# hagabbar/GenNet

Hardware: AMD Instinct MI355X
Metric: waveforms/sec (CNN+GAN step, 2048-sample BBH) (higher is better)
Workload: dtype f32

## Files before the change

### gennet_amd/csrc/capi.hip

```cpp
#include <stdarg.h>
#include <algorithm>
#include <mutex>
#include <vector>
#include <stdlib.h>
#include "common.h"

namespace gn {

static thread_local char g_err[512] = "";

void set_error(const char* fmt, ...) {
  va_list ap;
  va_start(ap, fmt);
  vsnprintf(g_err, sizeof(g_err), fmt, ap);
  va_end(ap);
}

int check_launch(const char* what) {
  hipError_t e = hipGetLastError();
  if (e != hipSuccess) {
    set_error("%s: %s", what, hipGetErrorString(e));
    return GN_ELAUNCH;
  }
  return GN_OK;
}

struct ProfRec {
  hipEvent_t a, b;
  double flop;
  int kind;
  double bytes;
};
static bool g_prof_on = false;
static std::vector<ProfRec> g_prof;
static std::vector<hipEvent_t> g_pool;
static hipEvent_t g_cur;
static std::mutex g_prof_mu;

static hipEvent_t get_event() {
  if (!g_pool.empty()) {
    hipEvent_t e = g_pool.back();
    g_pool.pop_back();
    return e;
  }
  hipEvent_t e;
  (void)hipEventCreate(&e);
  return e;
}

static thread_local const uint64_t* g_rng_base = nullptr;
const uint64_t* rng_base() { return g_rng_base; }

void prof_begin(hipStream_t s) {
  if (!g_prof_on) return;
  g_cur = get_event();
  (void)hipEventRecord(g_cur, s);
}

void prof_end(hipStream_t s, double flop, int kind, double bytes) {
  if (!g_prof_on) return;
  hipEvent_t b = get_event();
  (void)hipEventRecord(b, s);
  std::lock_guard<std::mutex> lk(g_prof_mu);
  g_prof.push_back({g_cur, b, flop, kind, bytes});
}

const Switches& switches() {
  static const Switches sw = [] {
    auto on = [](const char* name) { return getenv(name) != nullptr; };
    const char* gflop = getenv("GN_BF16X3_MIN_GFLOP");
    return Switches{on("GN_CONV_NOPIPE"),  on("GN_CONV_NODMA"),   on("GN_CONV_NOMERGE"),    on("GN_CONV_NONARROW"), on("GN_CONV_NOPATCH"),
                    on("GN_WGRAD_NOPIPE"), on("GN_BF16X3_NO_MERGE"), gflop ? atof(gflop) : 50.0};
  }();
  return sw;
}

static int g_conv_math = 0;
static void* g_conv_ws = nullptr;
static size_t g_conv_ws_bytes = 0;
constexpr size_t kWinoKernelBytes = 64ull << 20;

static bool split_worth_it(int B, int M, int ntaps, int Cin, int Cout) {
  constexpr int min_cin = 256, min_cout = 256;
  return Cin >= min_cin && Cout >= min_cout && 2.0 * B * (double)M * ntaps * Cin * Cout >= switches().bf16x3_min_gflop * 1e9;
}
static bool split_worth_it(const ConvArgs& a, int w_taps) {
  return w_taps > 0 ? split_worth_it(a.B, (a.Ly + 1) / 2, w_taps, a.Cin, a.Cout) : split_worth_it(a.B, a.M, a.t.ntaps, a.Cin, a.Cout);
}

static bool needs_any(int Cin, int Cout) {
  const bool strict = Cin <= 4 ? Cout % 4 == 0 : Cout <= 4 ? Cin % 4 == 0 : (Cin % 4 == 0 && Cout % 4 == 0);
  return !strict;
}

enum ConvFamily { CONV_SMALL, CONV_WINO, CONV_WINO_S2, CONV_BF16X3, CONV_DIRECT, CONV_ANYC };

static ConvFamily select_conv(const ConvArgs& a, int w_taps) {
  if (a.any_channels && needs_any(a.Cin, a.Cout)) return CONV_ANYC;
  if (a.Cin <= 4 || a.Cout <= 4) return CONV_SMALL;
  if (g_conv_math == 2 && a.Cin >= 32 && conv_wino_supported(a) && conv_wino_workspace_bytes(a.Cin, a.Cout) <= kWinoKernelBytes) return CONV_WINO;
  if (g_conv_math == 2 && conv_wino_s2_kind(a) == 1 && conv_wino_s2_workspace_bytes(a.Cin, a.Cout) <= kWinoKernelBytes) return CONV_WINO_S2;
  if (g_conv_math == 1 && split_worth_it(a, w_taps) && conv_bf16x3_supported(a)) return CONV_BF16X3;
  return CONV_DIRECT;
}

enum DgradFamily { DGRAD_WINO_S2, DGRAD_BF16X3_MERGED, DGRAD_MERGED, DGRAD_PHASES };

static DgradFamily select_dgrad(const ConvArgs& a) {
  if (a.any_channels && needs_any(a.Cin, a.Cout)) return DGRAD_PHASES;
  if (a.Ly < 2 || a.Cin <= 4 || a.Cout <= 4) return DGRAD_PHASES;
  if (g_conv_math == 2 && conv_wino_s2_kind(a) == 2 && conv_wino_s2_workspace_bytes(a.Cin, a.Cout) <= kWinoKernelBytes) return DGRAD_WINO_S2;
  const Switches& sw = switches();
  const bool split = g_conv_math == 1 && split_worth_it(a, 5);
  if (split) return !sw.bf16x3_no_merge && conv_bf16x3_merged_kind(a) ? DGRAD_BF16X3_MERGED : DGRAD_PHASES;
  if (!sw.conv_nomerge && !sw.conv_nopipe && !sw.conv_nodma && conv_pipe_merged_supported(a)) return DGRAD_MERGED;
  return DGRAD_PHASES;
}

enum WgradFamily { WGRAD_SMALL, WGRAD_WINO, WGRAD_WINO_S2, WGRAD_BF16X3, WGRAD_DIRECT, WGRAD_ANYC };

static WgradFamily select_wgrad(const WgradArgs& a) {
  if (a.any_channels && needs_any(a.Cin, a.Cout)) return WGRAD_ANYC;
  if (a.Cin <= 4 || a.Cout <= 4) return WGRAD_SMALL;
  if (g_conv_math == 2 && wgrad_wino_supported(a) && conv_wino_workspace_bytes(a.Cin, a.Cout) <= kWinoKernelBytes) return WGRAD_WINO;
  if (g_conv_math == 2 && wgrad_wino_s2_supported(a) && conv_wino_s2_workspace_bytes(a.Cin, a.Cout) <= kWinoKernelBytes) return WGRAD_WINO_S2;
  if (g_conv_math == 1 && split_worth_it(a.B, a.M, a.ntaps, a.Cin, a.Cout) && wgrad_bf16x3_supported(a)) return WGRAD_BF16X3;
  return WGRAD_DIRECT;
}

static size_t wgrad_ws_need(WgradFamily f, const WgradArgs& a) {
  switch (f) {
    case WGRAD_SMALL: return needs_any(a.Cin, a.Cout) ? 0 : wgrad_small_workspace_bytes(a.B, a.M, a.Cin, a.Cout, a.ntaps);
    case WGRAD_WINO: return wgrad_wino_workspace_bytes(a.B, a.M, a.Cin, a.Cout);
    case WGRAD_WINO_S2: return wgrad_wino_s2_workspace_bytes(a.B, a.M, a.Cin, a.Cout);
    case WGRAD_ANYC: return wgrad_anyc_workspace_bytes(a.B, a.M, a.Cin, a.Cout, a.ntaps);
    default: return wgrad_workspace_bytes(a.B, a.M, a.Cin, a.Cout, a.ntaps);
  }
}

static int ws_check(const char* what, size_t need, size_t have) {
  if (need <= have) return GN_OK;
  set_error("%s workspace: the selected kernel needs %zu bytes, the workspace has %zu", what, need, have);
  return GN_EWORKSPACE;
}

struct Phases { int w_taps; bool have_split; };

static int conv_run(const ConvArgs& a, hipStream_t s, Phases* ph = nullptr) {
  const ConvFamily f = select_conv(a, ph ? ph->w_taps : 0);
  int w_taps = ph ? ph->w_taps : 0;
  for (int j = 0; !ph && j < a.t.ntaps; ++j) w_taps = std::max(w_taps, a.t.widx[j] + 1);
  const size_t need = f == CONV_WINO ? conv_wino_workspace_bytes(a.Cin, a.Cout) : f == CONV_WINO_S2 ? conv_wino_s2_workspace_bytes(a.Cin, a.Cout)
                      : f == CONV_BF16X3 ? conv_bf16x3_workspace_bytes(a.B, a.Lin, a.Cin, a.Cout, w_taps) : 0;
  if (int rc = ws_check("conv-math", need, g_conv_ws_bytes)) return rc;
  switch (f) {
    case CONV_SMALL: return a.Cin <= 4 ? conv_smallcin_dispatch(a, s) : conv_smallcout_dispatch(a, s);
    case CONV_WINO: return conv_wino_run(a, g_conv_ws, g_conv_ws_bytes, s);
    case CONV_WINO_S2: return conv_wino_s2_run(a, g_conv_ws, g_conv_ws_bytes, s);
    case CONV_BF16X3:
      if (!(ph && ph->have_split)) {
        int rc = conv_bf16x3_split(a, w_taps, g_conv_ws, g_conv_ws_bytes, true, true, s);
        if (rc) return rc;
        if (ph) ph->have_split = true;
      }
      return conv_bf16x3_run(a, w_taps, g_conv_ws, s);
    case CONV_ANYC: return conv_anyc_dispatch(a, s);
    default: return conv_mfma_dispatch(a, s);
  }
}

static ConvArgs fwd_args(const float* x, const float* w, const float* bias, float* y, int B, int L, int Cin, int Cout, int k, int stride, int pad_left,
                         int Lout, int act, float act_param) {
  ConvArgs a = {};
  a.x = x; a.w = w; a.bias = bias; a.y = y;
  a.B = B; a.Lin = L; a.Cin = Cin; a.Cout = Cout; a.M = Lout; a.Ly = Lout;
  a.t.ntaps = k; a.t.in_stride = stride; a.t.out_stride = 1;
  for (int j = 0; j < k; ++j) { a.t.off[j] = j - pad_left; a.t.widx[j] = j; }
  a.act = act; a.act_param = act_param;
  return a;
}

static int set_conv_math_impl(int mode, void* workspace, size_t workspace_bytes) {
  GN_REQUIRE(mode >= 0 && mode <= 2, "set_conv_math: mode %d (0 = direct fp32, 1 = bf16x3, 2 = transform-domain fp32)", mode);
  GN_REQUIRE(mode == 0 || workspace, "set_conv_math: modes 1 and 2 need a device workspace");
  if (mode == 2 && workspace_bytes < kWinoKernelBytes) {
    set_error("set_conv_math: the transform-domain math needs a workspace of %zu bytes, got %zu", kWinoKernelBytes, workspace_bytes);
    return GN_EWORKSPACE;
  }
  g_conv_math = mode;
  g_conv_ws = mode ? workspace : nullptr;
  g_conv_ws_bytes = mode ? workspace_bytes : 0;
  return GN_OK;
}

__global__ void colsum_anyc_kernel(const float* __restrict__ x, double* __restrict__ acc, size_t n, int C) {
  double s[4] = {0, 0, 0, 0};
  const size_t stride = (size_t)gridDim.x * blockDim.x;
  for (size_t i = (size_t)blockIdx.x * blockDim.x + threadIdx.x; i < n; i += stride) {
    const int c = (int)(i % C);
    const double v = (double)x[i];
    s[0] += c == 0 ? v : 0.0; s[1] += c == 1 ? v : 0.0; s[2] += c == 2 ? v : 0.0; s[3] += c == 3 ? v : 0.0;
  }
  __shared__ double red[4][256];
  for (int c = 0; c < 4; ++c) red[c][threadIdx.x] = s[c];
  __syncthreads();
  for (int sft = 128; sft >= 1; sft >>= 1) {
    if (threadIdx.x < sft)
      for (int c = 0; c < 4; ++c) red[c][threadIdx.x] += red[c][threadIdx.x + sft];
    __syncthreads();
  }
  if (threadIdx.x < C) atomicAdd(&acc[threadIdx.x], red[threadIdx.x][0]);
}
__global__ void f64_to_f32_small_kernel(const double* __restrict__ a, float* __restrict__ o, int n) {
  if ((int)threadIdx.x < n) o[threadIdx.x] = (float)a[threadIdx.x];
}

static int bias_grad(const float* dy, float* db, size_t rows, int C, void* ws, size_t ws_bytes, hipStream_t s) {
  if (C % 4 == 0 || C > 4) {
    ColRedArgs r = {};
    r.a = dy; r.rows = rows; r.C = C;
    return colred_run(0, r, ws, ws_bytes, nullptr, db, s);
  }
  if (ws_bytes < 32) { set_error("bias_grad: workspace too small"); return GN_EWORKSPACE; }
  (void)hipMemsetAsync(ws, 0, 32, s);
  size_t g = (rows * C + 255) / 256;
  if (g > 1024) g = 1024;
  hipLaunchKernelGGL(colsum_anyc_kernel, dim3((unsigned)g), dim3(256), 0, s, dy, (double*)ws, rows * C, C);
  hipLaunchKernelGGL(f64_to_f32_small_kernel, dim3(1), dim3(64), 0, s, (const double*)ws, db, C);
  return check_launch("bias_grad");
}

static size_t bias_grad_ws(size_t rows, int C) { return C % 4 == 0 || C > 4 ? colred_workspace_bytes(rows, C) : 32; }

__global__ __launch_bounds__(256) void dense_any_kernel(const float* __restrict__ A, const float* __restrict__ Bm, const float* __restrict__ bias,
                                                        float* __restrict__ C, int M, int N, int K, size_t sam, size_t sak, size_t sbk, size_t sbn, int act,
                                                        float p) {
  __shared__ float As[16][17], Bs[16][17];
  const int tx = threadIdx.x % 16, ty = threadIdx.x / 16;
  const int m = blockIdx.y * 16 + ty, n = blockIdx.x * 16 + tx;
  float acc = 0.f;
  for (int k0 = 0; k0 < K; k0 += 16) {
    const int ka = k0 + tx, kb = k0 + ty;
    As[ty][tx] = (m < M && ka < K) ? A[(size_t)m * sam + (size_t)ka * sak] : 0.f;
    Bs[ty][tx] = (kb < K && n < N) ? Bm[(size_t)kb * sbk + (size_t)n * sbn] : 0.f;
    __syncthreads();
#pragma unroll
    for (int kk = 0; kk < 16; ++kk) acc = fmaf(As[ty][kk], Bs[kk][tx], acc);
    __syncthreads();
  }
  if (m < M && n < N) C[(size_t)m * N + n] = act_apply(bias ? acc + bias[n] : acc, act, p);
}
static int dense_any_gemm(const float* A, const float* Bm, const float* bias, float* C, int M, int N, int K, size_t sam, size_t sak, size_t sbk, size_t sbn,
                          int act, float p, hipStream_t s) {
  if (M <= 0 || N <= 0) return GN_OK;
  if ((M + 15) / 16 > 65535) { set_error("dense: %d rows exceed the grid", M); return GN_EINVAL; }
  hipLaunchKernelGGL(dense_any_kernel, dim3(cdiv(N, 16), cdiv(M, 16)), dim3(256), 0, s, A, Bm, bias, C, M, N, K, sam, sak, sbk, sbn, act, p);
  return check_launch("dense_any");
}
static bool dense_any_shape(int in, int out) { return (in % 4 || out % 4) && !(out <= 4 && in % 4 == 0); }

}

using namespace gn;

extern "C" {

const char* gn_last_error(void) { return g_err; }
int gn_version(void) { return 100; }

int gn_prof_enable(int on) {
  g_prof_on = on != 0;
  return GN_OK;
}
int gn_prof_reset(void) {
  std::lock_guard<std::mutex> lk(g_prof_mu);
  for (auto& r : g_prof) {
    g_pool.push_back(r.a);
    g_pool.push_back(r.b);
  }
  g_prof.clear();
  return GN_OK;
}
int gn_prof_collect(int kind, double* out) {
  std::lock_guard<std::mutex> lk(g_prof_mu);
  double ms = 0, flop = 0, cnt = 0, bytes = 0;
  for (auto& r : g_prof) {
    if (kind >= 0 && r.kind != kind) continue;
    cnt += 1;
    if (hipEventSynchronize(r.b) != hipSuccess) { set_error("prof: event sync failed"); return GN_ELAUNCH; }
    float t = 0;
    if (hipEventElapsedTime(&t, r.a, r.b) != hipSuccess) { set_error("prof: elapsed failed"); return GN_ELAUNCH; }
    ms += t;
    flop += r.flop;
    bytes += r.bytes;
  }
  out[0] = cnt;
  out[1] = ms;
  out[2] = flop;
  out[3] = bytes;
  return GN_OK;
}

static int fwd_impl(const float* x, const float* w, const float* bias, float* y, int B, int L, int Cin, int Cout, int k, int stride, int pad_left, int Lout,
                    int act, float act_param, bool any_channels, void* stream) {
  GN_REQUIRE(x && w && y, "conv1d_fwd: null pointer");
  GN_REQUIRE(B >= 0 && L > 0 && Cin > 0 && Cout > 0 && k >= 1 && k <= 8 && stride >= 1 && Lout > 0, "conv1d_fwd: bad shape");
  GN_REQUIRE(pad_left >= 0 && stride * (Lout - 1) + k - pad_left <= L + k, "conv1d_fwd: Lout %d inconsistent with L %d k %d stride %d", Lout, L, k, stride);
  if (B == 0) return GN_OK;
  ConvArgs a = fwd_args(x, w, bias, y, B, L, Cin, Cout, k, stride, pad_left, Lout, act, act_param);
  a.any_channels = any_channels;
  return conv_run(a, (hipStream_t)stream);
}

int gn_conv1d_fwd(const float* x, const float* w, const float* bias, float* y, int B, int L, int Cin, int Cout, int k, int stride, int pad_left, int Lout,
                  int act, float act_param, void* stream) {
  return fwd_impl(x, w, bias, y, B, L, Cin, Cout, k, stride, pad_left, Lout, act, act_param, false, stream);
}
int gn_conv1d_fwd_any(const float* x, const float* w, const float* bias, float* y, int B, int L, int Cin, int Cout, int k, int stride, int pad_left, int Lout,
                      int act, float act_param, void* stream) {
  return fwd_impl(x, w, bias, y, B, L, Cin, Cout, k, stride, pad_left, Lout, act, act_param, true, stream);
}
int gn_conv1d_needs_any(int Cin, int Cout) { return needs_any(Cin, Cout) ? 1 : 0; }

int gn_set_conv_math(int mode, void* workspace, size_t workspace_bytes) { return set_conv_math_impl(mode, workspace, workspace_bytes); }

size_t gn_conv1d_bf16x3_workspace(int B, int L, int Cin, int Cout, int k) { return conv_bf16x3_workspace_bytes(B, L, Cin, Cout, k); }

size_t gn_conv1d_fwd_stats_workspace(int B, int Lout, int Cout) {
  const size_t fused = (size_t)B * (size_t)((Lout + 63) / 64) * 2 * (size_t)Cout * sizeof(double);
  const size_t plain = colred_workspace_bytes((size_t)B * Lout, Cout);
  return (fused > plain ? fused : plain) + 256;
}

int gn_conv1d_fwd_stats(const float* x, const float* w, const float* bias, float* y, double* sums, void* ws, size_t ws_bytes, int B, int L, int Cin, int Cout, int k,
                        int stride, int pad_left, int Lout, void* stream) {
  hipStream_t s = (hipStream_t)stream;
  GN_REQUIRE(x && w && y && sums && ws, "conv1d_fwd_stats: null pointer");
  GN_REQUIRE(B > 0 && L > 0 && Cin > 0 && Cout > 0 && Cout % 4 == 0 && k >= 1 && k <= 8 && stride >= 1 && Lout > 0, "conv1d_fwd_stats: bad shape");
  GN_REQUIRE(pad_left >= 0 && stride * (Lout - 1) + k - pad_left <= L + k, "conv1d_fwd_stats: Lout %d inconsistent with L %d k %d stride %d", Lout, L, k, stride);
  GN_REQUIRE(ws_bytes >= gn_conv1d_fwd_stats_workspace(B, Lout, Cout), "conv1d_fwd_stats: workspace too small");
  ConvArgs a = fwd_args(x, w, bias, y, B, L, Cin, Cout, k, stride, pad_left, Lout, GN_ACT_LINEAR, 0.f);
  int done = 0;
  a.stat_part = (double*)ws; a.stat_sums = sums; a.stat_done = &done;
  int rc = conv_run(a, s);
  if (rc || done) return rc;
  ColRedArgs r = {};
  r.a = y; r.rows = (size_t)B * Lout; r.C = Cout;
  return colred_run(1, r, ws, ws_bytes, sums, nullptr, s);
}

int gn_conv1d_fwd_bf16x3(const float* x, const float* w, const float* bias, float* y, void* ws, size_t ws_bytes, int B, int L, int Cin, int Cout, int k, int stride,
                         int pad_left, int Lout, int act, float act_param, int resplit, void* stream) {
  GN_REQUIRE(x && w && y && ws, "conv1d_fwd_bf16x3: null pointer");
  GN_REQUIRE(B >= 0 && L > 0 && Cin > 0 && Cout > 0 && k >= 1 && k <= 5 && stride >= 1 && Lout > 0 && pad_left >= 0, "conv1d_fwd_bf16x3: bad shape");
  if (B == 0) return GN_OK;
  ConvArgs a = fwd_args(x, w, bias, y, B, L, Cin, Cout, k, stride, pad_left, Lout, act, act_param);
  GN_REQUIRE(conv_bf16x3_supported(a), "conv1d_fwd_bf16x3: needs Cin %% 16 == 0, Cout %% 64 == 0, k <= 5, stride 1");
  if (resplit) {
    int rc = conv_bf16x3_split(a, k, ws, ws_bytes, true, true, (hipStream_t)stream);
    if (rc) return rc;
  }
  return conv_bf16x3_run(a, k, ws, (hipStream_t)stream);
}

size_t gn_conv1d_wino_workspace(int Cin, int Cout) { return conv_wino_workspace_bytes(Cin, Cout); }

int gn_conv1d_fwd_wino(const float* x, const float* w, const float* bias, float* y, void* ws, size_t ws_bytes, int B, int L, int Cin, int Cout, int k, int stride,
                       int pad_left, int Lout, int act, float act_param, void* stream) {
  GN_REQUIRE(x && w && y && ws, "conv1d_fwd_wino: null pointer");
  GN_REQUIRE(B >= 0 && L > 0 && Cin > 0 && Cout > 0 && k == 5 && stride == 1 && Lout > 0 && pad_left >= 0, "conv1d_fwd_wino: 5 taps, unit stride");
  if (B == 0) return GN_OK;
  ConvArgs a = fwd_args(x, w, bias, y, B, L, Cin, Cout, k, stride, pad_left, Lout, act, act_param);
  return conv_wino_run(a, ws, ws_bytes, (hipStream_t)stream);
}

int gn_conv1d_fwd_dropout(const float* x, const float* w, const float* bias, const uint8_t* mask, float* y, int B, int L, int Cin, int Cout, int k, int stride,
                          int pad_left, int Lout, int act, float act_param, float rate, void* stream) {
  GN_REQUIRE(x && w && y && mask, "conv1d_fwd_dropout: null pointer");
  GN_REQUIRE(B >= 0 && L > 0 && Cin > 0 && Cout > 4 && Cout % 4 == 0 && k >= 1 && k <= 5 && stride >= 1 && Lout > 0 && pad_left >= 0, "conv1d_fwd_dropout: bad shape");
  GN_REQUIRE(rate >= 0.f && rate < 1.f, "conv1d_fwd_dropout: bad rate %f", rate);
  if (B == 0) return GN_OK;
  ConvArgs a = fwd_args(x, w, bias, y, B, L, Cin, Cout, k, stride, pad_left, Lout, act, act_param);
  a.mask = mask; a.keep_scale = 1.0f / (1.0f - rate);
  return conv_run(a, (hipStream_t)stream);
}

int gn_conv1d_transpose_w(const float* w, float* wt, int k, int Cin, int Cout, void* stream) {
  GN_REQUIRE(w && wt && k >= 1 && Cin > 0 && Cout > 0, "transpose_w: bad arguments");
  return transpose_w(w, wt, k, Cin, Cout, (hipStream_t)stream);
}

static int dgrad_impl(const float* dy, const float* wt, float* dx, int B, int L, int Cin, int Cout, int k, int stride, int pad_left, int Lout, const float* gy,
                      const uint8_t* gmask, int gact, float gparam, float grate, void* stream, bool any_channels = false) {
  GN_REQUIRE(dy && wt && dx, "conv1d_dgrad: null pointer");
  GN_REQUIRE(B >= 0 && L > 0 && Cin > 0 && Cout > 0 && k >= 1 && k <= 8 && stride >= 1 && Lout > 0 && pad_left >= 0, "conv1d_dgrad: bad shape");
  if (B == 0) return GN_OK;
  auto phase_args = [&](int p) {
    ConvArgs a = {};
    a.x = dy; a.w = wt; a.bias = nullptr; a.y = dx;
    a.B = B; a.Lin = Lout; a.Cin = Cout; a.Cout = Cin; a.Ly = L;
    a.t.in_stride = 1; a.t.out_stride = stride;
    a.act = GN_ACT_LINEAR;
    a.any_channels = any_channels;
    a.gy = gy; a.gmask = gmask; a.gact = gact; a.gparam = gparam; a.gscale = 1.0f / (1.0f - grate);
    a.M = (L - std::max(p, 0) + stride - 1) / stride;
    a.t.out_off = p < 0 ? pad_left & 1 : p;
    if (p < 0) a.t.out_off_odd = 1 - (pad_left & 1);
    for (int kk = 0; kk < k; ++kk) {
      const int d = (p < 0 ? (kk + pad_left) & 1 : p) + pad_left - kk;
      if (((d % stride) + stride) % stride) continue;
      a.t.off[a.t.ntaps] = (d >= 0) ? d / stride : -((-d) / stride);
      a.t.widx[a.t.ntaps++] = kk;
    }
    return a;
  };
  hipStream_t s = (hipStream_t)stream;
  if (stride == 2 && k == 5) {
    const ConvArgs a = phase_args(-1);
    const DgradFamily f = select_dgrad(a);
    const size_t need = f == DGRAD_WINO_S2 ? conv_wino_s2_workspace_bytes(a.Cin, a.Cout)
                        : f == DGRAD_BF16X3_MERGED ? conv_bf16x3_workspace_bytes(a.B, a.Lin, a.Cin, a.Cout, 5) : 0;
    if (int rc = ws_check("conv-math", need, g_conv_ws_bytes)) return rc;
    if (f == DGRAD_WINO_S2) return conv_wino_s2_run(a, g_conv_ws, g_conv_ws_bytes, s);
    if (f == DGRAD_MERGED) return conv_pipe_run_merged(a, s);
    if (f == DGRAD_BF16X3_MERGED) {
      int rc = conv_bf16x3_split(a, 5, g_conv_ws, g_conv_ws_bytes, true, true, s);
      return rc ? rc : conv_bf16x3_run_merged(a, g_conv_ws, s);
    }
  }
  Phases ph = {stride > 1 ? k : 0, false};
  for (int p = 0; p < stride && p < L; ++p) {
    const ConvArgs a = phase_args(p);
    GN_REQUIRE(a.t.ntaps > 0, "conv1d_dgrad: phase %d has no taps (k %d < stride %d)", p, k, stride);
    int rc = conv_run(a, s, stride > 1 ? &ph : nullptr);
    if (rc) return rc;
  }
  return GN_OK;
}

int gn_conv1d_dgrad(const float* dy, const float* wt, float* dx, int B, int L, int Cin, int Cout, int k, int stride, int pad_left, int Lout, void* stream) {
  return dgrad_impl(dy, wt, dx, B, L, Cin, Cout, k, stride, pad_left, Lout, nullptr, nullptr, GN_ACT_LINEAR, 0.f, 0.f, stream);
}

int gn_conv1d_dgrad_any(const float* dy, const float* wt, float* dx, int B, int L, int Cin, int Cout, int k, int stride, int pad_left, int Lout, void* stream) {
  return dgrad_impl(dy, wt, dx, B, L, Cin, Cout, k, stride, pad_left, Lout, nullptr, nullptr, GN_ACT_LINEAR, 0.f, 0.f, stream, true);
}

int gn_conv1d_dgrad_fused(const float* dy, const float* wt, float* dx, int B, int L, int Cin, int Cout, int k, int stride, int pad_left, int Lout,
                          const float* y_prev, const uint8_t* mask_prev, int act_prev, float act_param_prev, float rate_prev, void* stream) {
  GN_REQUIRE(y_prev, "conv1d_dgrad_fused: y_prev is NULL");
  GN_REQUIRE(Cin > 4 && Cout > 4, "conv1d_dgrad_fused: only the MFMA path fuses the producer's activation gradient (Cin %d, Cout %d)", Cin, Cout);
  GN_REQUIRE(rate_prev >= 0.f && rate_prev < 1.f, "conv1d_dgrad_fused: bad rate");
  return dgrad_impl(dy, wt, dx, B, L, Cin, Cout, k, stride, pad_left, Lout, y_prev, mask_prev, act_prev, act_param_prev, mask_prev ? rate_prev : 0.f, stream);
}

static WgradArgs wgrad_args(const float* x, const float* dy, void* ws, int B, int L, int Cin, int Cout, int k, int stride, int pad_left, int Lout) {
  WgradArgs a = {};
  a.x = x; a.dy = dy; a.part = (float*)ws;
  a.B = B; a.Lin = L; a.Cin = Cin; a.Cout = Cout; a.M = Lout; a.ntaps = k; a.in_stride = stride;
  for (int j = 0; j < k && j < 8; ++j) a.off[j] = j - pad_left;
  return a;
}

size_t gn_conv1d_wgrad_workspace(int B, int L, int Cin, int Cout, int k, int stride, int Lout) {
  WgradArgs a = wgrad_args(nullptr, nullptr, nullptr, B, L, Cin, Cout, k, stride, 0, Lout);
  a.any_channels = 1;
  return std::max(wgrad_ws_need(select_wgrad(a), a), bias_grad_ws((size_t)B * Lout, Cout)) + 256;
}

static int wgrad_impl(const float* x, const float* dy, float* dw, float* db, void* ws, size_t ws_bytes, int B, int L, int Cin, int Cout, int k, int stride,
                      int pad_left, int Lout, bool any_channels, void* stream) {
  GN_REQUIRE(x && dy && dw && ws, "conv1d_wgrad: null pointer");
  GN_REQUIRE(B > 0 && L > 0 && Cin > 0 && Cout > 0 && k >= 1 && k <= 5 && stride >= 1 && Lout > 0 && pad_left >= 0, "conv1d_wgrad: bad shape");
  hipStream_t s = (hipStream_t)stream;
  WgradArgs a = wgrad_args(x, dy, ws, B, L, Cin, Cout, k, stride, pad_left, Lout);
  a.db = db;
  a.any_channels = any_channels;
  const WgradFamily f = select_wgrad(a);
  int rc = ws_check("conv1d_wgrad", wgrad_ws_need(f, a), ws_bytes);
  if (rc) return rc;
  switch (f) {
    case WGRAD_SMALL: {
      WgradSmallArgs sa = {x, dy, (float*)ws, B, L, Cin, Cout, Lout, k, stride};
      std::copy(a.off, a.off + k, sa.off);
      rc = wgrad_small_dispatch(sa, dw, ws_bytes, s);
      break;
    }
    case WGRAD_WINO: rc = wgrad_wino_run(a, dw, s); break;
    case WGRAD_WINO_S2: rc = wgrad_wino_s2_run(a, dw, s); break;
    case WGRAD_ANYC: rc = wgrad_anyc_dispatch(a, dw, ws_bytes, s); break;
    case WGRAD_BF16X3:
      rc = ws_check("conv-math", wgrad_bf16x3_workspace_bytes(B, Lout, Cin, Cout, stride), g_conv_ws_bytes);
      if (!rc) rc = wgrad_bf16x3_dispatch(a, dw, g_conv_ws, g_conv_ws_bytes, s);
      break;
    default:
      rc = wgrad_mfma_dispatch(a, dw, ws_bytes, s);
      if (!rc && a.db_done) return GN_OK;
  }
  if (rc) return rc;
  return db ? bias_grad(dy, db, (size_t)B * Lout, Cout, ws, ws_bytes, s) : GN_OK;
}

int gn_conv1d_wgrad(const float* x, const float* dy, float* dw, float* db, void* ws, size_t ws_bytes, int B, int L, int Cin, int Cout, int k, int stride,
                    int pad_left, int Lout, void* stream) {
  return wgrad_impl(x, dy, dw, db, ws, ws_bytes, B, L, Cin, Cout, k, stride, pad_left, Lout, false, stream);
}
int gn_conv1d_wgrad_any(const float* x, const float* dy, float* dw, float* db, void* ws, size_t ws_bytes, int B, int L, int Cin, int Cout, int k, int stride,
                        int pad_left, int Lout, void* stream) {
  return wgrad_impl(x, dy, dw, db, ws, ws_bytes, B, L, Cin, Cout, k, stride, pad_left, Lout, true, stream);
}

int gn_conv2d_w2_fold(const float* w, const float* bias, float* wf, float* biasf, int kh, int Cin, int Cout, void* stream) {
  GN_REQUIRE(w && wf && kh >= 1 && Cin > 0 && Cout > 0, "conv2d_w2_fold: bad arguments");
  return conv2d_w2_fold(w, bias, wf, biasf, kh, Cin, Cout, (hipStream_t)stream);
}
int gn_conv2d_w2_unfold_grad(const float* dwf, const float* dbf, float* dw, float* db, int kh, int Cin, int Cout, void* stream) {
  GN_REQUIRE(dwf && dw && kh >= 1 && Cin > 0 && Cout > 0, "conv2d_w2_unfold_grad: bad arguments");
  return conv2d_w2_unfold(dwf, dbf, dw, db, kh, Cin, Cout, (hipStream_t)stream);
}
int gn_conv1d_up2_fold(const float* w, const float* bias, float* wf, float* biasf, int Cin, int Cout, int stride, void* stream) {
  GN_REQUIRE(w && wf && Cin > 0 && Cout > 0 && (stride == 1 || stride == 2), "conv1d_up2_fold: bad arguments (5-tap 'same' conv, stride 1 or 2)");
  return up2_fold(w, bias, wf, biasf, Cin, Cout, stride, (hipStream_t)stream);
}
int gn_conv1d_up2_unfold_grad(const float* dwf, const float* dbf, float* dw, float* db, int Cin, int Cout, int stride, void* stream) {
  GN_REQUIRE(dwf && dw && Cin > 0 && Cout > 0 && (stride == 1 || stride == 2) && (!db || dbf), "conv1d_up2_unfold_grad: bad arguments");
  return up2_unfold(dwf, dbf, dw, db, Cin, Cout, stride, (hipStream_t)stream);
}

size_t gn_bias_grad_workspace(size_t rows, int C) { return bias_grad_ws(rows, C) + 256; }

int gn_bias_grad(const float* dy, float* db, void* ws, size_t ws_bytes, size_t rows, int C, void* stream) {
  GN_REQUIRE(dy && db && ws && rows > 0 && C > 0, "bias_grad: bad arguments");
  return bias_grad(dy, db, rows, C, ws, ws_bytes, (hipStream_t)stream);
}

int gn_dense_fwd(const float* x, const float* w, const float* bias, float* y, int B, int in, int out, int act, float act_param, void* stream) {
  GN_REQUIRE(x && w && y && B >= 0 && in > 0 && out > 0, "dense_fwd: bad arguments");
  if (B == 0) return GN_OK;
  if (dense_any_shape(in, out))
    return dense_any_gemm(x, w, bias, y, B, out, in, (size_t)in, 1, (size_t)out, 1, act, act_param, (hipStream_t)stream);
  if (out <= 4) return dense_small_fwd(x, w, bias, y, B, in, out, act, act_param, (hipStream_t)stream);
  return conv_mfma_dispatch(fwd_args(x, w, bias, y, 1, B, in, out, 1, 1, 0, B, act, act_param), (hipStream_t)stream);
}

size_t gn_dense_bwd_workspace(int B, int in, int out) {
  if (out <= 4) return 256;
  if (dense_any_shape(in, out)) return bias_grad_ws((size_t)B, out) + 256;
  size_t w = wgrad_workspace_bytes(1, B, in, out, 1);
  size_t b = bias_grad_ws((size_t)B, out);
  return (w > b ? w : b) + (size_t)in * out * sizeof(float) + 256;
}

int gn_dense_bwd_fused(const float* x, const float* w, const float* dy, float* dx, float* dw, float* db, int B, int in, int out, const uint8_t* mask_prev,
                       int act_prev, float act_param_prev, float rate_prev, void* stream) {
  GN_REQUIRE(x && w && dy && dx && dw && B > 0 && in > 0 && out >= 1 && out <= 4, "dense_bwd_fused: bad arguments (small-output heads only)");
  GN_REQUIRE(rate_prev >= 0.f && rate_prev < 1.f, "dense_bwd_fused: bad rate");
  return dense_small_bwd(x, w, dy, dx, dw, db, B, in, out, (hipStream_t)stream, act_prev, act_param_prev, mask_prev, 1.0f / (1.0f - (mask_prev ? rate_prev : 0.f)));
}

int gn_dense_bwd(const float* x, const float* w, const float* dy, float* dx, float* dw, float* db, void* ws, size_t ws_bytes, int B, int in, int out, void* stream) {
  GN_REQUIRE(x && w && dy && dw && B > 0 && in > 0 && out > 0, "dense_bwd: bad arguments");
  hipStream_t s = (hipStream_t)stream;
  if (dense_any_shape(in, out)) {
    GN_REQUIRE(ws && ws_bytes >= bias_grad_ws((size_t)B, out), "dense_bwd: workspace too small");
    int rc = dx ? dense_any_gemm(dy, w, nullptr, dx, B, in, out, (size_t)out, 1, 1, (size_t)out, GN_ACT_LINEAR, 0.f, s) : GN_OK;
    if (!rc) rc = dense_any_gemm(x, dy, nullptr, dw, in, out, B, 1, (size_t)in, (size_t)out, 1, GN_ACT_LINEAR, 0.f, s);
    if (!rc && db) rc = bias_grad(dy, db, (size_t)B, out, ws, ws_bytes, s);
    return rc;
  }
  if (out <= 4) return dense_small_bwd(x, w, dy, dx, dw, db, B, in, out, s);
  GN_REQUIRE(ws && ws_bytes >= gn_dense_bwd_workspace(B, in, out), "dense_bwd: workspace too small");
  const size_t wt_bytes = (size_t)in * out * sizeof(float);
  float* wt = (float*)ws;
  void* ws2 = (char*)ws + wt_bytes;
  const size_t ws2_bytes = ws_bytes - wt_bytes;
  int rc;
  if (dx) {
    rc = transpose_w(w, wt, 1, in, out, s);
    if (rc) return rc;
    rc = conv_run(fwd_args(dy, wt, nullptr, dx, 1, B, out, in, 1, 1, 0, B, GN_ACT_LINEAR, 0.f), s);
    if (rc) return rc;
  }
  WgradArgs g = wgrad_args(x, dy, ws2, 1, B, in, out, 1, 1, 0, B);
  rc = wgrad_mfma_dispatch(g, dw, ws2_bytes, s);
  if (rc) return rc;
  if (db) rc = bias_grad(dy, db, (size_t)B, out, ws2, ws2_bytes, s);
  return rc;
}

int gn_act_fwd(const float* x, float* y, size_t n, int act, float p, void* stream) {
  GN_REQUIRE(x && y, "act_fwd: null pointer");
  return act_fwd(x, y, n, act, p, (hipStream_t)stream);
}
int gn_act_bwd(const float* dy, const float* y, float* dx, size_t n, int act, float p, void* stream) {
  GN_REQUIRE(dy && y && dx, "act_bwd: null pointer");
  return act_bwd(dy, y, dx, n, act, p, (hipStream_t)stream);
}
int gn_act_dropout_bwd(const float* dy, const float* y, const uint8_t* mask, float* dx, size_t n, int act, float p, float rate, void* stream) {
  GN_REQUIRE(dy && y && mask && dx && rate >= 0.f && rate < 1.f, "act_dropout_bwd: bad arguments");
  return act_dropout_bwd(dy, y, mask, dx, n, act, p, rate, (hipStream_t)stream);
}
int gn_dropout_mask(uint8_t* mask, size_t n, float rate, uint64_t seed, uint64_t offset, void* stream) {
  GN_REQUIRE(mask && rate >= 0.f && rate < 1.f, "dropout_mask: bad arguments");
  return dropout_mask(mask, n, rate, seed, offset, (hipStream_t)stream);
}
int gn_dropout_apply(const float* x, const uint8_t* mask, float* y, size_t n, float rate, void* stream) {
  GN_REQUIRE(x && mask && y && rate >= 0.f && rate < 1.f, "dropout_apply: bad arguments");
  return dropout_apply(x, mask, y, n, rate, (hipStream_t)stream);
}
int gn_upsample2_fwd(const float* x, float* y, int B, int L, int C, void* stream) {
  GN_REQUIRE(x && y, "upsample2_fwd: null pointer");
  return upsample2_fwd(x, y, B, L, C, (hipStream_t)stream);
}
int gn_upsample2_bwd(const float* dy, float* dx, int B, int L, int C, void* stream) {
  GN_REQUIRE(dy && dx, "upsample2_bwd: null pointer");
  return upsample2_bwd(dy, dx, B, L, C, (hipStream_t)stream);
}
int gn_subtract_stack_fwd(const float* x, const float* event, float* img, int B, int n, void* stream) {
  GN_REQUIRE(x && event && img, "subtract_stack_fwd: null pointer");
  return subtract_stack_fwd(x, event, img, B, n, (hipStream_t)stream);
}
int gn_subtract_stack_bwd(const float* dimg, float* dx, int B, int n, void* stream) {
  GN_REQUIRE(dimg && dx, "subtract_stack_bwd: null pointer");
  return subtract_stack_bwd(dimg, dx, B, n, (hipStream_t)stream);
}
int gn_affine_stack_fwd(const float* x, const float* b0, const float* b1, float a0, float a1, float* img, int B, int n, void* stream) {
  GN_REQUIRE(x && img && B >= 0 && n > 0, "affine_stack_fwd: bad arguments");
  return affine_stack_fwd(x, b0, b1, a0, a1, img, B, n, (hipStream_t)stream);
}
int gn_affine_stack_bwd(const float* dimg, float a0, float a1, float* dx, int B, int n, void* stream) {
  GN_REQUIRE(dimg && dx && B >= 0 && n > 0, "affine_stack_bwd: bad arguments");
  return affine_stack_bwd(dimg, a0, a1, dx, B, n, (hipStream_t)stream);
}
int gn_assemble_d_batch(const float* real, const float* noise, const float* fake, const float* event, float* sX, int B, int n, void* stream) {
  GN_REQUIRE(real && noise && fake && event && sX && B >= 0 && n > 0, "assemble_d_batch: bad arguments");
  return assemble_d_batch(real, noise, fake, event, sX, B, n, (hipStream_t)stream);
}
int gn_fill_uniform(float* out, size_t n, float lo, float hi, uint64_t seed, uint64_t offset, void* stream) {
  GN_REQUIRE(out, "fill_uniform: null pointer");
  return fill_uniform(out, n, lo, hi, seed, offset, (hipStream_t)stream);
}
int gn_fill_normal(float* out, size_t n, float mean, float sd, uint64_t seed, uint64_t offset, void* stream) {
  GN_REQUIRE(out, "fill_normal: null pointer");
  return fill_normal(out, n, mean, sd, seed, offset, (hipStream_t)stream);
}
int gn_gaussian_noise_fwd(const float* x, float* y, size_t n, float stddev, uint64_t seed, uint64_t offset, void* stream) {
  GN_REQUIRE((x && y) || !n, "gaussian_noise_fwd: null pointer");
  return gaussian_noise_fwd(x, y, n, stddev, seed, offset, (hipStream_t)stream);
}
int gn_gaussian_dropout_apply(const float* x, float* y, size_t n, float sd, uint64_t seed, uint64_t offset, void* stream) {
  GN_REQUIRE((x && y) || !n, "gaussian_dropout_apply: null pointer");
  return gaussian_dropout_apply(x, y, n, sd, seed, offset, (hipStream_t)stream);
}
int gn_alpha_dropout_fwd(const float* x, float* y, size_t n, float rate, float a, float b, float alpha_p, uint64_t seed, uint64_t offset, void* stream) {
  GN_REQUIRE(((x && y) || !n) && rate > 0.f && rate < 1.f, "alpha_dropout_fwd: bad arguments");
  return alpha_dropout_fwd(x, y, n, rate, a, b, alpha_p, seed, offset, (hipStream_t)stream);
}
int gn_alpha_dropout_bwd(const float* dy, float* dx, size_t n, float rate, float a, uint64_t seed, uint64_t offset, void* stream) {
  GN_REQUIRE(((dy && dx) || !n) && rate > 0.f && rate < 1.f, "alpha_dropout_bwd: bad arguments");
  return alpha_dropout_bwd(dy, dx, n, rate, a, seed, offset, (hipStream_t)stream);
}
int gn_gather_rows(const float* src, const int64_t* idx, float* out, int rows, int width, void* stream) {
  GN_REQUIRE(src && idx && out && rows >= 0 && width > 0, "gather_rows: bad arguments");
  return gather_rows(src, idx, out, rows, width, (hipStream_t)stream);
}
int gn_axpy(float* y, const float* x, float a, size_t n, void* stream) {
  GN_REQUIRE(y && x, "axpy: null pointer");
  return axpy(y, x, a, n, (hipStream_t)stream);
}

size_t gn_bn_stats_workspace(size_t rows, int C) { return colred_workspace_bytes(rows, C) + 256; }

int gn_bn_stats(const float* x, size_t rows, int C, double* sums, void* ws, size_t ws_bytes, void* stream) {
  GN_REQUIRE(x && sums && ws && rows > 0 && C > 0, "bn_stats: bad arguments");
  ColRedArgs r = {};
  r.a = x; r.rows = rows; r.C = C;
  return colred_run(1, r, ws, ws_bytes, sums, nullptr, (hipStream_t)stream);
}
int gn_bn_finalize(const double* sums, double count, const float* gamma, const float* beta, float eps, float momentum, float* moving_mean, float* moving_var,
                   float* scale, float* shift, float* save_mean, float* save_invstd, int C, void* stream) {
  GN_REQUIRE(sums && gamma && beta && scale && shift && save_mean && save_invstd && C > 0 && count > 1.0, "bn_finalize: bad arguments");
  GN_REQUIRE((moving_mean == nullptr) == (moving_var == nullptr), "bn_finalize: moving_mean/moving_var must both be given or both be NULL");
  return bn_finalize(sums, count, gamma, beta, eps, momentum, moving_mean, moving_var, nullptr, nullptr, 0.f, scale, shift, save_mean, save_invstd, C,
                     (hipStream_t)stream);
}

int gn_bn_finalize_zero_debias(const double* sums, double count, const float* gamma, const float* beta, float eps, float momentum, float* moving_mean,
                               float* moving_var, float* biased_mean, float* biased_var, int local_step, float* scale, float* shift, float* save_mean,
                               float* save_invstd, int C, void* stream) {
  GN_REQUIRE(sums && gamma && beta && scale && shift && save_mean && save_invstd && C > 0 && count > 1.0, "bn_finalize_zero_debias: bad arguments");
  GN_REQUIRE(moving_mean && moving_var && biased_mean && biased_var && local_step >= 1,
             "bn_finalize_zero_debias: needs moving_mean/var, the biased accumulators and the incremented local_step (>= 1, got %d)", local_step);
  return bn_finalize(sums, count, gamma, beta, eps, momentum, moving_mean, moving_var, biased_mean, biased_var, (float)local_step, scale, shift, save_mean,
                     save_invstd, C, (hipStream_t)stream);
}
int gn_bn_infer_coeffs(const float* gamma, const float* beta, const float* moving_mean, const float* moving_var, float eps, float* scale, float* shift, int C,
                       void* stream) {
  GN_REQUIRE(gamma && beta && moving_mean && moving_var && scale && shift && C > 0, "bn_infer_coeffs: bad arguments");
  return bn_infer_coeffs(gamma, beta, moving_mean, moving_var, eps, scale, shift, C, (hipStream_t)stream);
}
int gn_bn_apply(const float* x, const float* scale, const float* shift, const uint8_t* mask, float* y, size_t rows, int C, int act, float p, float rate,
                void* stream) {
  GN_REQUIRE(x && scale && shift && y && C > 0, "bn_apply: bad arguments");
  GN_REQUIRE(rate >= 0.f && rate < 1.f && (mask || rate == 0.f), "bn_apply: dropout rate %f without mask", rate);
  return bn_apply(x, scale, shift, mask, y, rows, C, act, p, mask ? rate : 0.f, (hipStream_t)stream);
}
int gn_bn_bwd_stats(const float* dy, const float* y, const float* x, const uint8_t* mask, const float* save_mean, const float* save_invstd, double* dsums, void* ws,
                    size_t ws_bytes, size_t rows, int C, int act, float p, float rate, const float* scale, const float* shift, void* stream) {
  GN_REQUIRE(dy && x && save_mean && save_invstd && dsums && ws && rows > 0 && C > 0, "bn_bwd_stats: bad arguments");
  GN_REQUIRE((scale == nullptr) == (shift == nullptr) && (y || scale), "bn_bwd_stats: needs the layer output y, or scale AND shift to recompute it");
  ColRedArgs r = {};
  r.a = dy; r.y = y; r.xpre = x; r.mask = mask; r.mean = save_mean; r.invstd = save_invstd; r.scale = scale; r.shift = shift;
  r.rows = rows; r.C = C; r.act = act; r.act_param = p; r.keep_scale = 1.0f / (1.0f - (mask ? rate : 0.f));
  return colred_run(2, r, ws, ws_bytes, dsums, nullptr, (hipStream_t)stream);
}
int gn_bn_bwd_apply(const float* dy, const float* y, const float* x, const uint8_t* mask, const float* gamma, const float* save_mean, const float* save_invstd,
                    const double* dsums_global, double count, const double* dsums_local, float* dx, float* dgamma, float* dbeta, size_t rows, int C, int act,
                    float p, float rate, const float* scale, const float* shift, void* stream) {
  GN_REQUIRE(dy && x && gamma && save_mean && save_invstd && dsums_global && dsums_local && dx && dgamma && dbeta && C > 0, "bn_bwd_apply: bad arguments");
  GN_REQUIRE((scale == nullptr) == (shift == nullptr) && (y || scale), "bn_bwd_apply: needs the layer output y, or scale AND shift to recompute it");
  return bn_bwd_apply(dy, y, x, mask, gamma, save_mean, save_invstd, dsums_global, count, dsums_local, dx, dgamma, dbeta, rows, C, act, p, mask ? rate : 0.f, scale,
                      shift, (hipStream_t)stream);
}

static int lazy_dy_check(const char* who, const float* g, const float* w, int L, int Lout, int k, int pad_left, size_t rows, int C, const float* scale,
                         const float* shift, LazyDy* z) {
  GN_REQUIRE(g && w && L > 0 && Lout > 0 && k >= 1 && k <= 5 && pad_left >= 0, "%s: bad conv description (1 filter, 1..5 taps, stride 1)", who);
  GN_REQUIRE(C % 4 == 0 && scale && shift, "%s: needs C %% 4 == 0 and the forward pass' scale / shift", who);
  GN_REQUIRE(rows % (size_t)L == 0 && rows / (size_t)L < 0x7fffffffull, "%s: rows %zu is not a whole number of length-%d segments", who, rows, L);
  z->g = g; z->w = w; z->L = L; z->Lout = Lout; z->k = k; z->pad_left = pad_left;
  return GN_OK;
}
int gn_bn_bwd_stats_conv1(const float* g, const float* w, int L, int Lout, int k, int pad_left, const float* x, const uint8_t* mask, const float* save_mean,
                          const float* save_invstd, double* dsums, void* ws, size_t ws_bytes, size_t rows, int C, int act, float p, float rate,
                          const float* scale, const float* shift, void* stream) {
  GN_REQUIRE(x && save_mean && save_invstd && dsums && ws && rows > 0 && C > 0, "bn_bwd_stats_conv1: bad arguments");
  ColRedArgs r = {};
  int rc = lazy_dy_check("bn_bwd_stats_conv1", g, w, L, Lout, k, pad_left, rows, C, scale, shift, &r.lz);
  if (rc) return rc;
  r.a = nullptr; r.y = nullptr; r.xpre = x; r.mask = mask; r.mean = save_mean; r.invstd = save_invstd; r.scale = scale; r.shift = shift;
  r.rows = rows; r.C = C; r.act = act; r.act_param = p; r.keep_scale = 1.0f / (1.0f - (mask ? rate : 0.f));
  return colred_run(2, r, ws, ws_bytes, dsums, nullptr, (hipStream_t)stream);
}
int gn_bn_bwd_apply_conv1(const float* g, const float* w, int L, int Lout, int k, int pad_left, const float* x, const uint8_t* mask, const float* gamma,
                          const float* save_mean, const float* save_invstd, const double* dsums_global, double count, const double* dsums_local, float* dx,
                          float* dgamma, float* dbeta, size_t rows, int C, int act, float p, float rate, const float* scale, const float* shift, void* stream) {
  GN_REQUIRE(x && gamma && save_mean && save_invstd && dsums_global && dsums_local && dx && dgamma && dbeta && C > 0, "bn_bwd_apply_conv1: bad arguments");
  LazyDy z = {};
  int rc = lazy_dy_check("bn_bwd_apply_conv1", g, w, L, Lout, k, pad_left, rows, C, scale, shift, &z);
  if (rc) return rc;
  return bn_bwd_apply(nullptr, nullptr, x, mask, gamma, save_mean, save_invstd, dsums_global, count, dsums_local, dx, dgamma, dbeta, rows, C, act, p,
                      mask ? rate : 0.f, scale, shift, (hipStream_t)stream, &z);
}

int gn_bce_loss(const float* p, const float* y, float* dp, float* out, int B, int Bglobal, void* stream) {
  GN_REQUIRE(p && y && dp && out, "bce_loss: null pointer");
  return loss_run(0, p, y, dp, out, B, Bglobal, (hipStream_t)stream);
}
int gn_mse_loss(const float* p, const float* y, float* dp, float* out, int B, int Bglobal, void* stream) {
  GN_REQUIRE(p && y && dp && out, "mse_loss: null pointer");
  return loss_run(1, p, y, dp, out, B, Bglobal, (hipStream_t)stream);
}
int gn_adam_step(float* p, const float* g, float* m, float* v, size_t n, float lr_t, float b1, float b2, float eps, void* stream) {
  GN_REQUIRE(p && g && m && v, "adam_step: null pointer");
  return adam_step(p, g, m, v, n, lr_t, b1, b2, eps, (hipStream_t)stream);
}

int gn_set_rng_base(const uint64_t* base_dev) {
  g_rng_base = base_dev;
  return GN_OK;
}
int gn_adam_step_dyn(float* p, const float* g, float* m, float* v, size_t n, const float* lr_t_dev, float b1, float b2, float eps, void* stream) {
  GN_REQUIRE(p && g && m && v && lr_t_dev, "adam_step_dyn: null pointer");
  return adam_step(p, g, m, v, n, 0.f, b1, b2, eps, (hipStream_t)stream, lr_t_dev);
}
int gn_optim_step(int rule, float* p, const float* g, float* s0, float* s1, float* s2, size_t n, float lr, const float* lr_dev, float h0, float h1,
                  float eps, int nesterov, const float* clip_scale, float clipvalue, void* stream) {
  GN_REQUIRE(rule >= GN_OPT_SGD && rule <= GN_OPT_AMSGRAD, "optim_step: unknown rule %d", rule);
  if (!n) return GN_OK;
  const int ns = rule == GN_OPT_AMSGRAD ? 3 : (rule == GN_OPT_ADADELTA || rule == GN_OPT_ADAMAX || rule == GN_OPT_ADAM) ? 2 : 1;
  GN_REQUIRE(p && g && s0 && (ns < 2 || s1) && (ns < 3 || s2), "optim_step: null pointer (rule %d keeps %d state arrays)", rule, ns);
  GN_REQUIRE(eps >= 0.f && clipvalue >= 0.f && h0 >= 0.f && h1 >= 0.f, "optim_step: negative hyper-parameter");
  GN_REQUIRE(rule == GN_OPT_SGD || rule == GN_OPT_ADAGRAD || h0 <= 1.f, "optim_step: rho / beta_1 %g outside [0, 1]", h0);
  GN_REQUIRE((rule != GN_OPT_ADAMAX && rule != GN_OPT_ADAM && rule != GN_OPT_AMSGRAD) || h1 <= 1.f, "optim_step: beta_2 %g outside [0, 1]", h1);
  OptArgs a = {};
  a.p = p; a.g = g; a.s0 = s0; a.s1 = ns > 1 ? s1 : nullptr; a.s2 = ns > 2 ? s2 : nullptr; a.n = n;
  a.lr = lr; a.lr_dev = lr_dev; a.h0 = h0; a.h1 = h1; a.eps = eps; a.nesterov = nesterov ? 1 : 0; a.clip_scale = clip_scale; a.clipvalue = clipvalue;
  return optim_step(rule, a, (hipStream_t)stream);
}
size_t gn_optim_sumsq_slots(size_t n) { return optim_sumsq_slots(n); }
int gn_optim_sumsq(const float* g, size_t n, double* partials, void* stream) {
  GN_REQUIRE(partials && (g || !n), "optim_sumsq: null pointer");
  return optim_sumsq(g, n, partials, (hipStream_t)stream);
}
int gn_optim_clip_factor(const double* partials, size_t count, float clipnorm, float* factor, void* stream) {
  GN_REQUIRE(partials && factor && count > 0, "optim_clip_factor: null pointer or no partials");
  GN_REQUIRE(clipnorm > 0.f, "optim_clip_factor: clipnorm %g must be > 0", clipnorm);
  return optim_clip_factor(partials, count, clipnorm, factor, (hipStream_t)stream);
}
int gn_fill_normal_dyn(float* out, size_t n, float mean, const float* sd_dev, uint64_t seed, uint64_t offset, void* stream) {
  GN_REQUIRE(out && sd_dev, "fill_normal_dyn: null pointer");
  return fill_normal(out, n, mean, 0.f, seed, offset, (hipStream_t)stream, sd_dev);
}
int gn_bn_finalize_zero_debias_dyn(const double* sums, double count, const float* gamma, const float* beta, float eps, float momentum, float* moving_mean,
                                   float* moving_var, float* biased_mean, float* biased_var, const int32_t* local_step_dev, float* scale, float* shift,
                                   float* save_mean, float* save_invstd, int C, void* stream) {
  GN_REQUIRE(sums && gamma && beta && scale && shift && save_mean && save_invstd && C > 0 && count > 1.0, "bn_finalize_zero_debias_dyn: bad arguments");
  GN_REQUIRE(moving_mean && moving_var && biased_mean && biased_var && local_step_dev, "bn_finalize_zero_debias_dyn: needs moving statistics, accumulators, step");
  return bn_finalize(sums, count, gamma, beta, eps, momentum, moving_mean, moving_var, biased_mean, biased_var, 1.f, scale, shift, save_mean, save_invstd, C,
                     (hipStream_t)stream, local_step_dev);
}

}
```

### gennet_amd/csrc/common.h

```cpp
#pragma once
#include <hip/hip_runtime.h>
#include <stdint.h>
#include <stdio.h>
#include "../../include/gennet_hip.h"

#define GN_LDS_DMA_CLOBBER() asm volatile("" ::: "v0", "v1", "v2", "v3")
#define gn_buffer_load_lds(...) do { __builtin_amdgcn_raw_ptr_buffer_load_lds(__VA_ARGS__); GN_LDS_DMA_CLOBBER(); } while (0)
#define gn_global_load_lds(...) do { __builtin_amdgcn_global_load_lds(__VA_ARGS__); GN_LDS_DMA_CLOBBER(); } while (0)

namespace gn {

void set_error(const char* fmt, ...);
int check_launch(const char* what);

struct Switches {
  bool conv_nopipe, conv_nodma, conv_nomerge, conv_nonarrow, conv_nopatch;
  bool wgrad_nopipe, bf16x3_no_merge;
  double bf16x3_min_gflop;
};
const Switches& switches();

const uint64_t* rng_base();
void prof_begin(hipStream_t s);
void prof_end(hipStream_t s, double flop, int kind, double bytes = 0.0);


struct ConvTaps {
  int ntaps;
  int in_stride;
  int off[8];
  int widx[8];
  int out_stride, out_off;
  int out_off_odd;
};

struct ConvArgs {
  const float* x;
  const float* w;
  const float* bias;
  float* y;
  int B, Lin, Cin, Cout;
  int M;
  int Ly;
  ConvTaps t;
  int act;
  float act_param;
  int any_channels;
  const uint8_t* mask;
  float keep_scale;
  const float* gy;
  const uint8_t* gmask;
  int gact;
  float gparam, gscale;
  double* stat_part;
  double* stat_sums;
  int* stat_done;
};

struct WgradArgs {
  const float* x;
  const float* dy;
  float* part;
  int B, Lin, Cin, Cout, M;
  int ntaps, in_stride;
  int off[8];
  int chunks_per_split;
  double* db_part;
  float* db;
  int db_done;
  int any_channels;
};

struct WgradSmallArgs {
  const float* x;
  const float* dy;
  float* part;
  int B, Lin, Cin, Cout, M;
  int ntaps, in_stride;
  int off[8];
  int rows_per_chunk;
};

struct LazyDy {
  const float* g;
  const float* w;
  int L, Lout, k, pad_left;
};

struct ColRedArgs {
  const float* a;
  const float* y;
  const float* xpre;
  const uint8_t* mask;
  const float* mean;
  const float* invstd;
  const float* scale;
  const float* shift;
  double* part;
  size_t rows;
  int C;
  int rows_per_chunk;
  int act;
  float act_param;
  float keep_scale;
  LazyDy lz;
};

int conv_mfma_dispatch(const ConvArgs& a, hipStream_t s);
size_t wgrad_workspace_bytes(int B, int M, int Cin, int Cout, int ntaps);
int wgrad_mfma_dispatch(WgradArgs& a, float* dw, size_t ws_bytes, hipStream_t s);
int wgrad_bf16x3_dispatch(WgradArgs& a, float* dw, void* split_ws, size_t split_ws_bytes, hipStream_t s);
int conv_pipe_try(const ConvArgs& a, bool tall, hipStream_t s, bool* launched);
bool conv_pipe_merged_supported(const ConvArgs& a);
int conv_pipe_run_merged(const ConvArgs& a, hipStream_t s);
void wgrad_pipe_launch(const WgradArgs& a, dim3 grid, bool narrow, hipStream_t s);
size_t conv_bf16x3_workspace_bytes(int B, int Lin, int Cin, int Cout, int w_taps);
bool conv_bf16x3_supported(const ConvArgs& a);
int conv_bf16x3_split(const ConvArgs& a, int w_taps, void* ws, size_t ws_bytes, bool split_x, bool split_w, hipStream_t s);
int conv_bf16x3_run(const ConvArgs& a, int w_taps, void* ws, hipStream_t s);
int conv_bf16x3_merged_kind(const ConvArgs& a);
int conv_bf16x3_run_merged(const ConvArgs& a, void* ws, hipStream_t s);
size_t conv_wino_workspace_bytes(int Cin, int Cout);
bool conv_wino_supported(const ConvArgs& a);
int conv_wino_run(const ConvArgs& a, void* ws, size_t ws_bytes, hipStream_t s);
size_t conv_wino_s2_workspace_bytes(int Cin, int Cout);
int conv_wino_s2_kind(const ConvArgs& a);
int conv_wino_s2_run(const ConvArgs& a, void* ws, size_t ws_bytes, hipStream_t s);
void wgrad_split_plan(int B, int M, int Cin, int Cout, int TC, int TN, int* splits, int* chunks_per_split);
bool wgrad_wino_supported(const WgradArgs& a);
size_t wgrad_wino_workspace_bytes(int B, int M, int Cin, int Cout);
int wgrad_wino_run(WgradArgs& a, float* dw, hipStream_t s);
bool wgrad_wino_s2_supported(const WgradArgs& a);
size_t wgrad_wino_s2_workspace_bytes(int B, int M, int Cin, int Cout);
int wgrad_wino_s2_run(WgradArgs& a, float* dw, hipStream_t s);
size_t wgrad_bf16x3_workspace_bytes(int B, int M, int Cin, int Cout, int in_stride);
bool wgrad_bf16x3_supported(const WgradArgs& a);
int wgrad_bf16x3_run(const WgradArgs& a, int splits, void* ws, size_t ws_bytes, hipStream_t s);
int conv_anyc_dispatch(const ConvArgs& a, hipStream_t s);
size_t wgrad_anyc_workspace_bytes(int B, int M, int Cin, int Cout, int ntaps);
int wgrad_anyc_dispatch(WgradArgs& a, float* dw, size_t ws_bytes, hipStream_t s);
int conv_smallcin_dispatch(const ConvArgs& a, hipStream_t s);
int conv_smallcout_dispatch(const ConvArgs& a, hipStream_t s);
size_t wgrad_small_workspace_bytes(int B, int M, int Cin, int Cout, int ntaps);
int wgrad_small_dispatch(WgradSmallArgs a, float* dw, size_t ws_bytes, hipStream_t s);
int dense_small_fwd(const float* x, const float* w, const float* bias, float* y, int B, int in, int out, int act, float p, hipStream_t s);
int dense_small_bwd(const float* x, const float* w, const float* dy, float* dx, float* dw, float* db, int B, int in, int out, hipStream_t s,
                    int gact = 0, float gparam = 0.f, const uint8_t* gmask = nullptr, float gscale = 1.f);
int act_fwd(const float* x, float* y, size_t n, int act, float p, hipStream_t s);
int act_bwd(const float* dy, const float* y, float* dx, size_t n, int act, float p, hipStream_t s);
int act_dropout_bwd(const float* dy, const float* y, const uint8_t* mask, float* dx, size_t n, int act, float p, float rate, hipStream_t s);
int dropout_mask(uint8_t* mask, size_t n, float rate, uint64_t seed, uint64_t offset, hipStream_t s);
int dropout_apply(const float* x, const uint8_t* mask, float* y, size_t n, float rate, hipStream_t s);
int upsample2_fwd(const float* x, float* y, int B, int L, int C, hipStream_t s);
int upsample2_bwd(const float* dy, float* dx, int B, int L, int C, hipStream_t s);
int subtract_stack_fwd(const float* x, const float* ev, float* img, int B, int n, hipStream_t s);
int subtract_stack_bwd(const float* dimg, float* dx, int B, int n, hipStream_t s);
int affine_stack_fwd(const float* x, const float* b0, const float* b1, float a0, float a1, float* img, int B, int n, hipStream_t s);
int affine_stack_bwd(const float* dimg, float a0, float a1, float* dx, int B, int n, hipStream_t s);
int assemble_d_batch(const float* real, const float* noise, const float* fake, const float* ev, float* sX, int B, int n, hipStream_t s);
int gather_rows(const float* src, const int64_t* idx, float* out, int rows, int width, hipStream_t s);
int axpy(float* y, const float* x, float a, size_t n, hipStream_t s);
int fill_uniform(float* out, size_t n, float lo, float hi, uint64_t seed, uint64_t offset, hipStream_t s);
int fill_normal(float* out, size_t n, float mean, float sd, uint64_t seed, uint64_t offset, hipStream_t s, const float* sd_dev = nullptr);
int gaussian_noise_fwd(const float* x, float* y, size_t n, float stddev, uint64_t seed, uint64_t offset, hipStream_t s);
int gaussian_dropout_apply(const float* x, float* y, size_t n, float sd, uint64_t seed, uint64_t offset, hipStream_t s);
int alpha_dropout_fwd(const float* x, float* y, size_t n, float rate, float a, float b, float alpha_p, uint64_t seed, uint64_t offset, hipStream_t s);
int alpha_dropout_bwd(const float* dy, float* dx, size_t n, float rate, float a, uint64_t seed, uint64_t offset, hipStream_t s);
size_t colred_workspace_bytes(size_t rows, int C);
int colred_run(int mode, ColRedArgs a, void* ws, size_t ws_bytes, double* out_f64, float* out_f32, hipStream_t s);
int colred_finalize(const double* part, double* out_f64, size_t n, int chunks, hipStream_t s);
int colred_finalize_f32(const double* part, float* out_f32, size_t n, int chunks, hipStream_t s);
int bn_finalize(const double* sums, double count, const float* gamma, const float* beta, float eps, float momentum, float* mm, float* mv,
                float* bm, float* bv, float zd_step, float* scale, float* shift, float* smean, float* sinv, int C, hipStream_t s,
                const int32_t* zd_step_dev = nullptr);
int bn_infer_coeffs(const float* gamma, const float* beta, const float* mm, const float* mv, float eps, float* scale, float* shift, int C, hipStream_t s);
int bn_apply(const float* x, const float* scale, const float* shift, const uint8_t* mask, float* y, size_t rows, int C, int act, float p, float rate, hipStream_t s);
int bn_bwd_apply(const float* dy, const float* y, const float* x, const uint8_t* mask, const float* gamma, const float* mean, const float* invstd,
                 const double* dsums_global, double count, const double* dsums_local, float* dx, float* dgamma, float* dbeta, size_t rows, int C,
                 int act, float p, float rate, const float* scale, const float* shift, hipStream_t s, const LazyDy* lz = nullptr);
int loss_run(int kind, const float* p, const float* y, float* dp, float* out, int B, int Bglobal, hipStream_t s);
int adam_step(float* p, const float* g, float* m, float* v, size_t n, float lr_t, float b1, float b2, float eps, hipStream_t s, const float* lr_t_dev = nullptr);
struct OptArgs {
  float *p, *s0, *s1, *s2;
  const float* g;
  size_t n;
  float lr;
  const float* lr_dev;
  float h0, h1, eps;
  int nesterov;
  const float* clip_scale;
  float clipvalue;
};
int optim_step(int rule, const OptArgs& a, hipStream_t s);
size_t optim_sumsq_slots(size_t n);
int optim_sumsq(const float* g, size_t n, double* partials, hipStream_t s);
int optim_clip_factor(const double* partials, size_t count, float clipnorm, float* factor, hipStream_t s);
int transpose_w(const float* w, float* wt, int k, int Cin, int Cout, hipStream_t s);
int conv2d_w2_fold(const float* w, const float* bias, float* wf, float* bf, int kh, int Cin, int Cout, hipStream_t s);
int conv2d_w2_unfold(const float* dwf, const float* dbf, float* dw, float* db, int kh, int Cin, int Cout, hipStream_t s);
int up2_fold(const float* w, const float* bias, float* wf, float* bf, int Cin, int Cout, int stride, hipStream_t s);
int up2_unfold(const float* dwf, const float* dbf, float* dw, float* db, int Cin, int Cout, int stride, hipStream_t s);

static inline unsigned cdiv(size_t a, size_t b) { return (unsigned)((a + b - 1) / b); }
static inline unsigned stream_grid(size_t n_items, int block = 256) {
  size_t g = (n_items + block - 1) / block;
  if (g > 256 * 8) g = 256 * 8;
  if (g < 1) g = 1;
  return (unsigned)g;
}

static inline void allow_big_lds(const void* kernel, unsigned long long* done) {
  int dev = 0;
  (void)hipGetDevice(&dev);
  const unsigned long long bit = 1ull << (dev & 63);
  if (!(*done & bit)) {
    (void)hipFuncSetAttribute(kernel, hipFuncAttributeMaxDynamicSharedMemorySize, 160 * 1024);
    *done |= bit;
  }
}

#define GN_REQUIRE(cond, ...)            \
  do {                                   \
    if (!(cond)) {                       \
      gn::set_error(__VA_ARGS__);        \
      return GN_EINVAL;                  \
    }                                    \
  } while (0)

__device__ __forceinline__ float gn_tanhf(float x) {
  const float ax = fabsf(x);
  const float e = __builtin_amdgcn_exp2f(ax * 2.8853900817779268f);
  const float big = 1.f - 2.f * __builtin_amdgcn_rcpf(e + 1.f);
  const float x2 = ax * ax;
  float q = fmaf(x2, -1382.f / 155925.f, 62.f / 2835.f);
  q = fmaf(x2, q, -17.f / 315.f);
  q = fmaf(x2, q, 2.f / 15.f);
  q = fmaf(x2, q, -1.f / 3.f);
  const float small = fmaf(ax * x2, q, ax);
  return copysignf(ax < 0.35f ? small : big, x);
}

__device__ __forceinline__ float act_apply(float x, int act, float p) {
  switch (act) {
    case GN_ACT_RELU: return fmaxf(x, 0.f);
    case GN_ACT_RELU_MAX: return fminf(fmaxf(x, 0.f), p);
    case GN_ACT_LEAKY: return x > 0.f ? x : p * x;
    case GN_ACT_TANH: return gn_tanhf(x);
    case GN_ACT_SIGMOID: return 1.f / (1.f + expf(-x));
    default: return x;
  }
}

__device__ __forceinline__ float act_grad_from_y(float y, int act, float p) {
  switch (act) {
    case GN_ACT_RELU: return y > 0.f ? 1.f : 0.f;
    case GN_ACT_RELU_MAX: return (y > 0.f && y < p) ? 1.f : 0.f;
    case GN_ACT_LEAKY: return y > 0.f ? 1.f : p;
    case GN_ACT_TANH: return 1.f - y * y;
    case GN_ACT_SIGMOID: return y * (1.f - y);
    default: return 1.f;
  }
}

struct Philox4 {
  uint32_t v[4];
};

__host__ __device__ __forceinline__ uint32_t mulhi32(uint32_t a, uint32_t b) { return (uint32_t)(((uint64_t)a * b) >> 32); }

__host__ __device__ __forceinline__ Philox4 philox4x32_10(uint64_t counter, uint64_t seed) {
  uint32_t c0 = (uint32_t)counter, c1 = (uint32_t)(counter >> 32), c2 = 0, c3 = 0;
  uint32_t k0 = (uint32_t)seed, k1 = (uint32_t)(seed >> 32);
#pragma unroll
  for (int r = 0; r < 10; ++r) {
    const uint32_t M0 = 0xD2511F53u, M1 = 0xCD9E8D57u;
    uint32_t h0 = mulhi32(M0, c0), l0 = M0 * c0;
    uint32_t h1 = mulhi32(M1, c2), l1 = M1 * c2;
    uint32_t n0 = h1 ^ c1 ^ k0, n1 = l1, n2 = h0 ^ c3 ^ k1, n3 = l0;
    c0 = n0; c1 = n1; c2 = n2; c3 = n3;
    k0 += 0x9E3779B9u; k1 += 0xBB67AE85u;
  }
  Philox4 o;
  o.v[0] = c0; o.v[1] = c1; o.v[2] = c2; o.v[3] = c3;
  return o;
}

__host__ __device__ __forceinline__ float u01_24(uint32_t x) { return (float)(x >> 8) * (1.0f / 16777216.0f); }
__host__ __device__ __forceinline__ double u01_53(uint32_t hi, uint32_t lo) {
  uint64_t x = (((uint64_t)hi << 32) | lo) >> 11;
  return ((double)x + 0.5) * (1.0 / 9007199254740992.0);
}

}
```

### gennet_amd/csrc/small_conv.hip

```cpp
#include "common.h"

namespace gn {



constexpr int SMALLCIN_WIN = (2 * 255 + 5) * 4 + 4;

template <int CIN>
__global__ __launch_bounds__(256) void conv_smallcin_kernel(ConvArgs a, int m_tiles, int MT) {
  constexpr int MAXT = 5;
  const int NQ = a.Cout >> 2;
  const int NQc = NQ < 256 ? NQ : 256;
  const int RL = 256 / NQc;
  const int tid = threadIdx.x;
  const int q0 = tid % NQc, rl = tid / NQc;
  const int m_tile = blockIdx.x % m_tiles, b = blockIdx.x / m_tiles;
  const int m_lo = m_tile * MT, m_hi = min(a.M, m_lo + MT);
  const float* xb = a.x + (size_t)b * a.Lin * CIN;
  float* yb = a.y + (size_t)b * a.Ly * a.Cout;
  __shared__ float xw[SMALLCIN_WIN];
  int minoff = a.t.off[0], maxoff = a.t.off[0];
  for (int j = 1; j < a.t.ntaps; ++j) {
    minoff = min(minoff, a.t.off[j]);
    maxoff = max(maxoff, a.t.off[j]);
  }
  const int t_lo = a.t.in_stride * m_lo + minoff;
  const int n_win = (a.t.in_stride * (m_hi - 1 - m_lo) + (maxoff - minoff) + 1) * CIN;
  for (int idx = tid; idx < n_win; idx += 256) {
    const int t = t_lo + idx / CIN;
    xw[idx] = (t >= 0 && t < a.Lin) ? xb[(size_t)t * CIN + idx % CIN] : 0.f;
  }
  __syncthreads();
  if (rl >= RL) return;
  for (int q = q0; q < NQ; q += NQc) {
    float4 wv[MAXT][CIN];
#pragma unroll
    for (int j = 0; j < MAXT; ++j)
#pragma unroll
      for (int c = 0; c < CIN; ++c)
        wv[j][c] = j < a.t.ntaps ? *reinterpret_cast<const float4*>(a.w + ((size_t)a.t.widx[j] * CIN + c) * a.Cout + 4 * q) : make_float4(0.f, 0.f, 0.f, 0.f);
    float4 bias = make_float4(0.f, 0.f, 0.f, 0.f);
    if (a.bias) bias = *reinterpret_cast<const float4*>(a.bias + 4 * q);
#pragma unroll 4
    for (int m = m_lo + rl; m < m_hi; m += RL) {
      float4 s = bias;
#pragma unroll
      for (int j = 0; j < MAXT; ++j) {
        if (j >= a.t.ntaps) break;
        const float* xr = xw + (a.t.in_stride * m + a.t.off[j] - t_lo) * CIN;
#pragma unroll
        for (int c = 0; c < CIN; ++c) {
          const float xv = xr[c];
          s.x = fmaf(xv, wv[j][c].x, s.x); s.y = fmaf(xv, wv[j][c].y, s.y);
          s.z = fmaf(xv, wv[j][c].z, s.z); s.w = fmaf(xv, wv[j][c].w, s.w);
        }
      }
      s.x = act_apply(s.x, a.act, a.act_param); s.y = act_apply(s.y, a.act, a.act_param);
      s.z = act_apply(s.z, a.act, a.act_param); s.w = act_apply(s.w, a.act, a.act_param);
      const size_t o = (size_t)(a.t.out_stride * m + a.t.out_off) * a.Cout + 4 * q;
      if (a.mask) {
        const uchar4 k = *reinterpret_cast<const uchar4*>(a.mask + (size_t)b * a.Ly * a.Cout + o);
        s.x = k.x ? s.x * a.keep_scale : 0.f; s.y = k.y ? s.y * a.keep_scale : 0.f;
        s.z = k.z ? s.z * a.keep_scale : 0.f; s.w = k.w ? s.w * a.keep_scale : 0.f;
      }
      *reinterpret_cast<float4*>(yb + o) = s;
    }
  }
}

int conv_smallcin_dispatch(const ConvArgs& a, hipStream_t s) {
  if (a.Cin < 1 || a.Cin > 4 || a.Cout % 4 || a.t.ntaps > 5) {
    set_error("conv_smallcin: Cin %d (1..4) / Cout %d (%%4) / ntaps %d (<=5) unsupported", a.Cin, a.Cout, a.t.ntaps);
    return GN_EINVAL;
  }
  const int NQ = a.Cout / 4, NQc = NQ < 256 ? NQ : 256, RL = 256 / NQc;
  int MT = RL * 16 < 256 ? RL * 16 : 256;
  int minoff = a.t.off[0], maxoff = a.t.off[0];
  for (int j = 1; j < a.t.ntaps; ++j) {
    minoff = a.t.off[j] < minoff ? a.t.off[j] : minoff;
    maxoff = a.t.off[j] > maxoff ? a.t.off[j] : maxoff;
  }
  if (a.t.in_stride < 1) {
    set_error("conv_smallcin: in_stride %d < 1", a.t.in_stride);
    return GN_EINVAL;
  }
  auto window = [&](int mt) { return ((long long)a.t.in_stride * (mt - 1) + (maxoff - minoff) + 1) * a.Cin; };
  while (MT > 1 && window(MT) > SMALLCIN_WIN) MT >>= 1;
  if (window(MT) > SMALLCIN_WIN) {
    set_error("conv_smallcin: tap span %d x Cin %d does not fit the %d-float input window", maxoff - minoff + 1, a.Cin, SMALLCIN_WIN);
    return GN_EINVAL;
  }
  const int m_tiles = cdiv(a.M, MT);
  const unsigned grid = (unsigned)m_tiles * a.B;
  if (grid == 0) return GN_OK;
  switch (a.Cin) {
    case 1: hipLaunchKernelGGL(conv_smallcin_kernel<1>, dim3(grid), dim3(256), 0, s, a, m_tiles, MT); break;
    case 2: hipLaunchKernelGGL(conv_smallcin_kernel<2>, dim3(grid), dim3(256), 0, s, a, m_tiles, MT); break;
    case 3: hipLaunchKernelGGL(conv_smallcin_kernel<3>, dim3(grid), dim3(256), 0, s, a, m_tiles, MT); break;
    default: hipLaunchKernelGGL(conv_smallcin_kernel<4>, dim3(grid), dim3(256), 0, s, a, m_tiles, MT); break;
  }
  return check_launch("conv_smallcin");
}

template <int COUT>
__global__ __launch_bounds__(256) void conv_smallcout_kernel(ConvArgs a) {
  const int lane = threadIdx.x & 63;
  const size_t row = (size_t)blockIdx.x * 4 + (threadIdx.x >> 6);
  if (row >= (size_t)a.B * a.M) return;
  const int b = (int)(row / a.M), m = (int)(row % a.M);
  const float* xb = a.x + (size_t)b * a.Lin * a.Cin;
  float acc[COUT];
#pragma unroll
  for (int o = 0; o < COUT; ++o) acc[o] = 0.f;
  for (int j = 0; j < a.t.ntaps; ++j) {
    const int t = a.t.in_stride * m + a.t.off[j];
    if (t < 0 || t >= a.Lin) continue;
    const float* xr = xb + (size_t)t * a.Cin;
    const float* wj = a.w + (size_t)a.t.widx[j] * a.Cin * COUT;
    for (int c = 4 * lane; c < a.Cin; c += 256) {
      const float4 xv = *reinterpret_cast<const float4*>(xr + c);
      if (COUT == 1) {
        const float4 wv = *reinterpret_cast<const float4*>(wj + c);
        acc[0] = fmaf(xv.x, wv.x, acc[0]); acc[0] = fmaf(xv.y, wv.y, acc[0]);
        acc[0] = fmaf(xv.z, wv.z, acc[0]); acc[0] = fmaf(xv.w, wv.w, acc[0]);
      } else {
        const float xs[4] = {xv.x, xv.y, xv.z, xv.w};
#pragma unroll
        for (int e = 0; e < 4; ++e)
#pragma unroll
          for (int o = 0; o < COUT; ++o) acc[o] = fmaf(xs[e], wj[(size_t)(c + e) * COUT + o], acc[o]);
      }
    }
  }
#pragma unroll
  for (int o = 0; o < COUT; ++o) {
    float v = acc[o];
#pragma unroll
    for (int sft = 32; sft >= 1; sft >>= 1) v += __shfl_xor(v, sft, 64);
    acc[o] = v;
  }
  if (lane == 0) {
    float* yr = a.y + ((size_t)b * a.Ly + (size_t)(a.t.out_stride * m + a.t.out_off)) * COUT;
#pragma unroll
    for (int o = 0; o < COUT; ++o) yr[o] = act_apply(acc[o] + (a.bias ? a.bias[o] : 0.f), a.act, a.act_param);
  }
}

template <int NTAPS, int ROWS>
__global__ __launch_bounds__(256) void conv_cout1_rows_kernel(ConvArgs a, int runs_per_b) {
  const int lane = threadIdx.x & 63;
  const size_t run = (size_t)blockIdx.x * 4 + (threadIdx.x >> 6);
  if (run >= (size_t)a.B * runs_per_b) return;
  const int b = (int)(run / runs_per_b), m0 = (int)(run % runs_per_b) * ROWS;
  const float* xb = a.x + (size_t)b * a.Lin * a.Cin;
  const int t0 = m0 + a.t.off[0];
  float acc[ROWS];
#pragma unroll
  for (int r = 0; r < ROWS; ++r) acc[r] = 0.f;
  for (int c = 4 * lane; c < a.Cin; c += 256) {
    float4 wv[NTAPS];
#pragma unroll
    for (int j = 0; j < NTAPS; ++j) wv[j] = *reinterpret_cast<const float4*>(a.w + (size_t)a.t.widx[j] * a.Cin + c);
#pragma unroll
    for (int tl = 0; tl < ROWS + NTAPS - 1; ++tl) {
      const int t = t0 + tl;
      float4 xv = make_float4(0.f, 0.f, 0.f, 0.f);
      if (t >= 0 && t < a.Lin) xv = *reinterpret_cast<const float4*>(xb + (size_t)t * a.Cin + c);
#pragma unroll
      for (int j = 0; j < NTAPS; ++j) {
        const int r = tl - j;
        if (r >= 0 && r < ROWS) {
          acc[r] = fmaf(xv.x, wv[j].x, acc[r]); acc[r] = fmaf(xv.y, wv[j].y, acc[r]);
          acc[r] = fmaf(xv.z, wv[j].z, acc[r]); acc[r] = fmaf(xv.w, wv[j].w, acc[r]);
        }
      }
    }
  }
  float mine = 0.f;
#pragma unroll
  for (int r = 0; r < ROWS; ++r) {
    float v = acc[r];
#pragma unroll
    for (int sft = 32; sft >= 1; sft >>= 1) v += __shfl_xor(v, sft, 64);
    if (lane == r) mine = v;
  }
  if (lane < ROWS && m0 + lane < a.M)
    a.y[(size_t)b * a.Ly + (size_t)(m0 + lane + a.t.out_off)] = act_apply(mine + (a.bias ? a.bias[0] : 0.f), a.act, a.act_param);
}

int conv_smallcout_dispatch(const ConvArgs& a, hipStream_t s) {
  if (a.Cout < 1 || a.Cout > 4 || a.Cin % 4) {
    set_error("conv_smallcout: Cout %d (1..4) / Cin %d (%%4) unsupported", a.Cout, a.Cin);
    return GN_EINVAL;
  }
  const size_t rows = (size_t)a.B * a.M;
  if (rows == 0) return GN_OK;
  bool contiguous = a.t.in_stride == 1 && a.t.out_stride == 1 && a.t.ntaps == 5;
  for (int j = 1; j < a.t.ntaps; ++j) contiguous = contiguous && a.t.off[j] == a.t.off[0] + j;
  if (a.Cout == 1 && contiguous && a.Cin >= 256) {
    constexpr int ROWS = 16;
    const int runs_per_b = cdiv(a.M, ROWS);
    hipLaunchKernelGGL((conv_cout1_rows_kernel<5, ROWS>), dim3(cdiv((size_t)a.B * runs_per_b, 4)), dim3(256), 0, s, a, runs_per_b);
    return check_launch("conv_cout1_rows");
  }
  const unsigned grid = cdiv(rows, 4);
  switch (a.Cout) {
    case 1: hipLaunchKernelGGL(conv_smallcout_kernel<1>, dim3(grid), dim3(256), 0, s, a); break;
    case 2: hipLaunchKernelGGL(conv_smallcout_kernel<2>, dim3(grid), dim3(256), 0, s, a); break;
    case 3: hipLaunchKernelGGL(conv_smallcout_kernel<3>, dim3(grid), dim3(256), 0, s, a); break;
    default: hipLaunchKernelGGL(conv_smallcout_kernel<4>, dim3(grid), dim3(256), 0, s, a); break;
  }
  return check_launch("conv_smallcout");
}


template <int CS>
__global__ __launch_bounds__(256) void wgrad_smallcin_tab_kernel(WgradSmallArgs a) {
  constexpr int MAXT = 5, TR = 128, U = 4;
  const int NQ = a.Cout >> 2;
  const int NQc = NQ < 256 ? NQ : 256;
  const int RL = 256 / NQc;
  const int tid = threadIdx.x;
  const int ql = tid % NQc, rl = tid / NQc;
  const int q = blockIdx.x * NQc + ql;
  const bool active = (rl < RL) && (q < NQ);
  float4 acc[MAXT][CS];
#pragma unroll
  for (int j = 0; j < MAXT; ++j)
#pragma unroll
    for (int c = 0; c < CS; ++c) acc[j][c] = make_float4(0.f, 0.f, 0.f, 0.f);
  __shared__ float tab[TR][MAXT * CS];
  __shared__ float4 red[256];

  const size_t rows = (size_t)a.B * a.M;
  const size_t r_lo = (size_t)blockIdx.y * a.rows_per_chunk;
  const size_t r_hi = r_lo + a.rows_per_chunk < rows ? r_lo + a.rows_per_chunk : rows;
  const int per_row = a.ntaps * CS;
  for (size_t base = r_lo; base < r_hi; base += TR) {
    const int nr = (int)(r_hi - base < (size_t)TR ? r_hi - base : (size_t)TR);
    __syncthreads();
    for (int e = tid; e < nr * per_row; e += 256) {
      const int rr = e / per_row, jc = e % per_row;
      const int j = jc / CS, c = jc % CS;
      const size_t r = base + rr;
      const int b = (int)(r / a.M), m = (int)(r % a.M);
      const int t = a.in_stride * m + a.off[j];
      tab[rr][j * CS + c] = (t >= 0 && t < a.Lin) ? a.x[((size_t)b * a.Lin + t) * CS + c] : 0.f;
    }
    __syncthreads();
    if (active) {
      for (int r0 = rl; r0 < nr; r0 += RL * U) {
        float4 g[U];
#pragma unroll
        for (int u = 0; u < U; ++u) {
          const int rr = r0 + u * RL;
          g[u] = rr < nr ? *reinterpret_cast<const float4*>(a.dy + (base + rr) * a.Cout + 4 * q) : make_float4(0.f, 0.f, 0.f, 0.f);
        }
#pragma unroll
        for (int u = 0; u < U; ++u) {
          const int rr = r0 + u * RL;
          if (rr >= nr) break;
#pragma unroll
          for (int j = 0; j < MAXT; ++j) {
            if (j >= a.ntaps) break;
#pragma unroll
            for (int c = 0; c < CS; ++c) {
              const float xv = tab[rr][j * CS + c];
              acc[j][c].x = fmaf(xv, g[u].x, acc[j][c].x); acc[j][c].y = fmaf(xv, g[u].y, acc[j][c].y);
              acc[j][c].z = fmaf(xv, g[u].z, acc[j][c].z); acc[j][c].w = fmaf(xv, g[u].w, acc[j][c].w);
            }
          }
        }
      }
    }
  }
#pragma unroll
  for (int j = 0; j < MAXT; ++j) {
    if (j >= a.ntaps) break;
#pragma unroll
    for (int c = 0; c < CS; ++c) {
      __syncthreads();
      red[tid] = acc[j][c];
      __syncthreads();
      if (rl == 0 && q < NQ) {
        float4 s = red[ql];
        for (int k = 1; k < RL; ++k) {
          const float4 v = red[k * NQc + ql];
          s.x += v.x; s.y += v.y; s.z += v.z; s.w += v.w;
        }
        float* pc = a.part + (size_t)blockIdx.y * a.ntaps * a.Cin * a.Cout;
        *reinterpret_cast<float4*>(pc + ((size_t)j * CS + c) * a.Cout + 4 * q) = s;
      }
    }
  }
}

template <int CS, bool SMALL_IS_IN>
__global__ __launch_bounds__(256) void wgrad_small_kernel(WgradSmallArgs a) {
  constexpr int MAXT = 5;
  const int CL = SMALL_IS_IN ? a.Cout : a.Cin;
  const int NQ = CL >> 2;
  const int NQc = NQ < 256 ? NQ : 256;
  const int RL = 256 / NQc;
  const int tid = threadIdx.x;
  const int ql = tid % NQc, rl = tid / NQc;
  const int q = blockIdx.x * NQc + ql;
  const bool active = (rl < RL) && (q < NQ);
  float4 acc[MAXT][CS];
#pragma unroll
  for (int j = 0; j < MAXT; ++j)
#pragma unroll
    for (int c = 0; c < CS; ++c) acc[j][c] = make_float4(0.f, 0.f, 0.f, 0.f);

  const size_t rows = (size_t)a.B * a.M;
  const size_t r_lo = (size_t)blockIdx.y * a.rows_per_chunk;
  const size_t r_hi = r_lo + a.rows_per_chunk < rows ? r_lo + a.rows_per_chunk : rows;
  if (active) {
    for (size_t r = r_lo + rl; r < r_hi; r += RL) {
      const int b = (int)(r / a.M), m = (int)(r % a.M);
      if (SMALL_IS_IN) {
        const float4 g = *reinterpret_cast<const float4*>(a.dy + r * a.Cout + 4 * q);
#pragma unroll
        for (int j = 0; j < MAXT; ++j) {
          if (j >= a.ntaps) break;
          const int t = a.in_stride * m + a.off[j];
          if (t < 0 || t >= a.Lin) continue;
#pragma unroll
          for (int c = 0; c < CS; ++c) {
            const float xv = a.x[((size_t)b * a.Lin + t) * CS + c];
            acc[j][c].x = fmaf(xv, g.x, acc[j][c].x); acc[j][c].y = fmaf(xv, g.y, acc[j][c].y);
            acc[j][c].z = fmaf(xv, g.z, acc[j][c].z); acc[j][c].w = fmaf(xv, g.w, acc[j][c].w);
          }
        }
      } else {
        float gs[CS];
#pragma unroll
        for (int c = 0; c < CS; ++c) gs[c] = a.dy[r * CS + c];
#pragma unroll
        for (int j = 0; j < MAXT; ++j) {
          if (j >= a.ntaps) break;
          const int t = a.in_stride * m + a.off[j];
          if (t < 0 || t >= a.Lin) continue;
          const float4 xv = *reinterpret_cast<const float4*>(a.x + ((size_t)b * a.Lin + t) * a.Cin + 4 * q);
#pragma unroll
          for (int c = 0; c < CS; ++c) {
            acc[j][c].x = fmaf(xv.x, gs[c], acc[j][c].x); acc[j][c].y = fmaf(xv.y, gs[c], acc[j][c].y);
            acc[j][c].z = fmaf(xv.z, gs[c], acc[j][c].z); acc[j][c].w = fmaf(xv.w, gs[c], acc[j][c].w);
          }
        }
      }
    }
  }
  __shared__ float4 red[256];
#pragma unroll
  for (int j = 0; j < MAXT; ++j) {
    if (j >= a.ntaps) break;
#pragma unroll
    for (int c = 0; c < CS; ++c) {
      red[tid] = acc[j][c];
      __syncthreads();
      if (rl == 0 && q < NQ) {
        float4 s = red[ql];
        for (int k = 1; k < RL; ++k) {
          const float4 v = red[k * NQc + ql];
          s.x += v.x; s.y += v.y; s.z += v.z; s.w += v.w;
        }
        float* pc = a.part + (size_t)blockIdx.y * a.ntaps * a.Cin * a.Cout;
        if (SMALL_IS_IN) {
          *reinterpret_cast<float4*>(pc + ((size_t)j * CS + c) * a.Cout + 4 * q) = s;
        } else {
          float* d = pc + ((size_t)j * a.Cin + 4 * q) * CS + c;
          d[0] = s.x; d[CS] = s.y; d[2 * CS] = s.z; d[3 * CS] = s.w;
        }
      }
      __syncthreads();
    }
  }
}

template <int CS>
__global__ __launch_bounds__(256) void wgrad_smallcout_s1_kernel(WgradSmallArgs a) {
  constexpr int MAXT = 5, U = 4;
  const int NQ = a.Cin >> 2;
  const int NQc = NQ < 256 ? NQ : 256;
  const int RL = 256 / NQc;
  const int tid = threadIdx.x;
  const int ql = tid % NQc, rl = tid / NQc;
  const int q = blockIdx.x * NQc + ql;
  const bool active = (rl < RL) && (q < NQ);
  float4 acc[MAXT][CS];
#pragma unroll
  for (int j = 0; j < MAXT; ++j)
#pragma unroll
    for (int c = 0; c < CS; ++c) acc[j][c] = make_float4(0.f, 0.f, 0.f, 0.f);
  const size_t rows = (size_t)a.B * a.Lin;
  const size_t r_lo = (size_t)blockIdx.y * a.rows_per_chunk;
  const size_t r_hi = r_lo + a.rows_per_chunk < rows ? r_lo + a.rows_per_chunk : rows;
  constexpr int TR = 128;
  __shared__ float tab[TR][MAXT * CS];
  const int per_row = a.ntaps * CS;
  for (size_t base = r_lo; base < r_hi; base += TR) {
    const int nr = (int)(r_hi - base < (size_t)TR ? r_hi - base : (size_t)TR);
    __syncthreads();
    for (int e = tid; e < nr * per_row; e += 256) {
      const int rr = e / per_row, jc = e % per_row;
      const int j = jc / CS, c = jc % CS;
      const size_t r = base + rr;
      const int b = (int)(r / a.Lin), t = (int)(r % a.Lin);
      const int m = t - a.off[j];
      tab[rr][j * CS + c] = (m >= 0 && m < a.M) ? a.dy[((size_t)b * a.M + m) * CS + c] : 0.f;
    }
    __syncthreads();
    if (active) {
      for (int r0 = rl; r0 < nr; r0 += RL * U) {
        float4 xv[U];
#pragma unroll
        for (int u = 0; u < U; ++u) {
          const int rr = r0 + u * RL;
          xv[u] = rr < nr ? *reinterpret_cast<const float4*>(a.x + (base + rr) * a.Cin + 4 * q) : make_float4(0.f, 0.f, 0.f, 0.f);
        }
#pragma unroll
        for (int u = 0; u < U; ++u) {
          const int rr = r0 + u * RL;
          if (rr >= nr) break;
#pragma unroll
          for (int j = 0; j < MAXT; ++j) {
            if (j >= a.ntaps) break;
#pragma unroll
            for (int c = 0; c < CS; ++c) {
              const float g = tab[rr][j * CS + c];
              acc[j][c].x = fmaf(xv[u].x, g, acc[j][c].x); acc[j][c].y = fmaf(xv[u].y, g, acc[j][c].y);
              acc[j][c].z = fmaf(xv[u].z, g, acc[j][c].z); acc[j][c].w = fmaf(xv[u].w, g, acc[j][c].w);
            }
          }
        }
      }
    }
  }
  __syncthreads();
  __shared__ float4 red[256];
#pragma unroll
  for (int j = 0; j < MAXT; ++j) {
    if (j >= a.ntaps) break;
#pragma unroll
    for (int c = 0; c < CS; ++c) {
      red[tid] = acc[j][c];
      __syncthreads();
      if (rl == 0 && q < NQ) {
        float4 s = red[ql];
        for (int k = 1; k < RL; ++k) {
          const float4 v = red[k * NQc + ql];
          s.x += v.x; s.y += v.y; s.z += v.z; s.w += v.w;
        }
        float* d = a.part + (size_t)blockIdx.y * a.ntaps * a.Cin * a.Cout + ((size_t)j * a.Cin + 4 * q) * CS + c;
        d[0] = s.x; d[CS] = s.y; d[2 * CS] = s.z; d[3 * CS] = s.w;
      }
      __syncthreads();
    }
  }
}

static int wgrad_small_chunks(size_t rows, int CL) {
  const int NQ = CL / 4, NQc = NQ < 256 ? NQ : 256, RL = 256 / NQc;
  const int gx = (NQ + NQc - 1) / NQc;
  int chunks = (1024 + gx - 1) / gx;
  const size_t max_chunks = (rows + (size_t)RL * 8 - 1) / ((size_t)RL * 8);
  if ((size_t)chunks > max_chunks) chunks = (int)max_chunks;
  if (chunks < 1) chunks = 1;
  return chunks;
}

size_t wgrad_small_workspace_bytes(int B, int M, int Cin, int Cout, int ntaps) {
  const int CL = Cin <= 4 ? Cout : Cin;
  return (size_t)wgrad_small_chunks((size_t)B * M, CL) * ntaps * Cin * Cout * sizeof(float);
}

constexpr int SUM_GROUPS = 32;

__global__ void sum_partials_l1_kernel(float* __restrict__ part, size_t n, int chunks) {
  const size_t i = (size_t)blockIdx.x * blockDim.x + threadIdx.x;
  const int g = blockIdx.y;
  if (i >= n || g >= chunks) return;
  float s = part[(size_t)g * n + i];
  for (int k = g + SUM_GROUPS; k < chunks; k += SUM_GROUPS) s += part[(size_t)k * n + i];
  part[(size_t)g * n + i] = s;
}

__global__ void sum_partials_kernel(const float* __restrict__ part, float* __restrict__ out, size_t n, int chunks) {
  const size_t i = (size_t)blockIdx.x * blockDim.x + threadIdx.x;
  if (i >= n) return;
  float s = part[i];
  for (int k = 1; k < chunks; ++k) s += part[(size_t)k * n + i];
  out[i] = s;
}

static int sum_partials(float* part, float* out, size_t n, int chunks, hipStream_t s) {
  if (chunks > 2 * SUM_GROUPS) {
    hipLaunchKernelGGL(sum_partials_l1_kernel, dim3(cdiv(n, 256), SUM_GROUPS), dim3(256), 0, s, part, n, chunks);
    int rc = check_launch("sum_partials_l1");
    if (rc) return rc;
    chunks = SUM_GROUPS;
  }
  hipLaunchKernelGGL(sum_partials_kernel, dim3(cdiv(n, 256)), dim3(256), 0, s, part, out, n, chunks);
  return check_launch("wgrad_small_reduce");
}

int wgrad_small_dispatch(WgradSmallArgs a, float* dw, size_t ws_bytes, hipStream_t s) {
  const bool small_in = a.Cin <= 4;
  const int CS = small_in ? a.Cin : a.Cout, CL = small_in ? a.Cout : a.Cin;
  if (CS < 1 || CS > 4 || CL % 4 || a.ntaps > 5) {
    set_error("wgrad_small: Cin %d Cout %d ntaps %d unsupported", a.Cin, a.Cout, a.ntaps);
    return GN_EINVAL;
  }
  const size_t rows = (size_t)a.B * a.M;
  const int chunks = wgrad_small_chunks(rows, CL);
  if (ws_bytes < (size_t)chunks * a.ntaps * a.Cin * a.Cout * sizeof(float)) {
    set_error("wgrad_small: workspace too small");
    return GN_EWORKSPACE;
  }
  a.rows_per_chunk = (int)((rows + chunks - 1) / chunks);
  const int NQ = CL / 4, NQc = NQ < 256 ? NQ : 256;
  dim3 grid((NQ + NQc - 1) / NQc, chunks);
  if (!small_in && a.in_stride == 1) {
    a.rows_per_chunk = (int)(((size_t)a.B * a.Lin + chunks - 1) / chunks);
    switch (CS) {
      case 1: hipLaunchKernelGGL(wgrad_smallcout_s1_kernel<1>, grid, dim3(256), 0, s, a); break;
      case 2: hipLaunchKernelGGL(wgrad_smallcout_s1_kernel<2>, grid, dim3(256), 0, s, a); break;
      case 3: hipLaunchKernelGGL(wgrad_smallcout_s1_kernel<3>, grid, dim3(256), 0, s, a); break;
      default: hipLaunchKernelGGL(wgrad_smallcout_s1_kernel<4>, grid, dim3(256), 0, s, a); break;
    }
    int rc1 = check_launch("wgrad_smallcout_s1");
    if (rc1) return rc1;
    const size_t n1 = (size_t)a.ntaps * a.Cin * a.Cout;
    return sum_partials(a.part, dw, n1, chunks, s);
  }
#define GN_WS(CSV)                                                                                            \
  if (small_in) hipLaunchKernelGGL((wgrad_smallcin_tab_kernel<CSV>), grid, dim3(256), 0, s, a);               \
  else hipLaunchKernelGGL((wgrad_small_kernel<CSV, false>), grid, dim3(256), 0, s, a);
  switch (CS) {
    case 1: GN_WS(1); break;
    case 2: GN_WS(2); break;
    case 3: GN_WS(3); break;
    default: GN_WS(4); break;
  }
#undef GN_WS
  int rc = check_launch("wgrad_small");
  if (rc) return rc;
  const size_t n = (size_t)a.ntaps * a.Cin * a.Cout;
  return sum_partials(a.part, dw, n, chunks, s);
}

template <int OUT>
__global__ __launch_bounds__(1024) void dense_small_fwd_kernel(const float* __restrict__ x, const float* __restrict__ w, const float* __restrict__ bias,
                                                               float* __restrict__ y, int in, int act, float act_param) {
  const int b = blockIdx.x, tid = threadIdx.x;
  const float* xb = x + (size_t)b * in;
  float acc[OUT];
#pragma unroll
  for (int o = 0; o < OUT; ++o) acc[o] = 0.f;
  for (int i = 4 * tid; i < in; i += 4096) {
    const float4 xv = *reinterpret_cast<const float4*>(xb + i);
    if (OUT == 1) {
      const float4 wv = *reinterpret_cast<const float4*>(w + i);
      acc[0] = fmaf(xv.x, wv.x, acc[0]); acc[0] = fmaf(xv.y, wv.y, acc[0]);
      acc[0] = fmaf(xv.z, wv.z, acc[0]); acc[0] = fmaf(xv.w, wv.w, acc[0]);
    } else {
      const float xs[4] = {xv.x, xv.y, xv.z, xv.w};
#pragma unroll
      for (int e = 0; e < 4; ++e)
#pragma unroll
        for (int o = 0; o < OUT; ++o) acc[o] = fmaf(xs[e], w[(size_t)(i + e) * OUT + o], acc[o]);
    }
  }
  __shared__ float red[16][OUT];
#pragma unroll
  for (int o = 0; o < OUT; ++o) {
    float v = acc[o];
#pragma unroll
    for (int sft = 32; sft >= 1; sft >>= 1) v += __shfl_xor(v, sft, 64);
    if ((tid & 63) == 0) red[tid >> 6][o] = v;
  }
  __syncthreads();
  if (tid < OUT) {
    float v = 0.f;
    for (int k = 0; k < 16; ++k) v += red[k][tid];
    y[(size_t)b * OUT + tid] = act_apply(v + (bias ? bias[tid] : 0.f), act, act_param);
  }
}

int dense_small_fwd(const float* x, const float* w, const float* bias, float* y, int B, int in, int out, int act, float p, hipStream_t s) {
  if (out < 1 || out > 4 || in % 4) {
    set_error("dense_small_fwd: out %d (1..4) / in %d (%%4) unsupported", out, in);
    return GN_EINVAL;
  }
  if (B == 0) return GN_OK;
  switch (out) {
    case 1: hipLaunchKernelGGL(dense_small_fwd_kernel<1>, dim3(B), dim3(1024), 0, s, x, w, bias, y, in, act, p); break;
    case 2: hipLaunchKernelGGL(dense_small_fwd_kernel<2>, dim3(B), dim3(1024), 0, s, x, w, bias, y, in, act, p); break;
    case 3: hipLaunchKernelGGL(dense_small_fwd_kernel<3>, dim3(B), dim3(1024), 0, s, x, w, bias, y, in, act, p); break;
    default: hipLaunchKernelGGL(dense_small_fwd_kernel<4>, dim3(B), dim3(1024), 0, s, x, w, bias, y, in, act, p); break;
  }
  return check_launch("dense_small_fwd");
}

template <int OUT>
__global__ __launch_bounds__(256) void dense_small_bwd_kernel(const float* __restrict__ x, const float* __restrict__ w, const float* __restrict__ dy,
                                                              float* __restrict__ dx, float* __restrict__ dw, int B, int in, int gact, float gparam,
                                                              const uint8_t* __restrict__ gmask, float gscale) {
  const size_t i = ((size_t)blockIdx.x * 256 + threadIdx.x) * 4;
  if (i >= (size_t)in) return;
  float wv[4][OUT], acc[4][OUT];
#pragma unroll
  for (int e = 0; e < 4; ++e)
#pragma unroll
    for (int o = 0; o < OUT; ++o) {
      wv[e][o] = w[(i + e) * OUT + o];
      acc[e][o] = 0.f;
    }
  constexpr int U = 8;
  for (int b0 = 0; b0 < B; b0 += U) {
    float4 xq[U];
    uchar4 mq[U];
#pragma unroll
    for (int u = 0; u < U; ++u) {
      const int bb = min(b0 + u, B - 1);
      xq[u] = *reinterpret_cast<const float4*>(x + (size_t)bb * in + i);
      mq[u] = (dx && gmask) ? *reinterpret_cast<const uchar4*>(gmask + (size_t)bb * in + i) : make_uchar4(1, 1, 1, 1);
    }
#pragma unroll
    for (int u = 0; u < U; ++u) {
    const int b = b0 + u;
    if (b >= B) break;
    const float4 xv = xq[u];
    const float xs[4] = {xv.x, xv.y, xv.z, xv.w};
    float g[OUT];
#pragma unroll
    for (int o = 0; o < OUT; ++o) g[o] = dy[(size_t)b * OUT + o];
    float d[4] = {0.f, 0.f, 0.f, 0.f};
#pragma unroll
    for (int e = 0; e < 4; ++e)
#pragma unroll
      for (int o = 0; o < OUT; ++o) {
        acc[e][o] = fmaf(xs[e], g[o], acc[e][o]);
        d[e] = fmaf(g[o], wv[e][o], d[e]);
      }
    if (dx) {
      if (gact != GN_ACT_LINEAR || gmask) {
        const uint8_t k[4] = {mq[u].x, mq[u].y, mq[u].z, mq[u].w};
#pragma unroll
        for (int e = 0; e < 4; ++e) d[e] = k[e] ? d[e] * gscale * act_grad_from_y(xs[e] / gscale, gact, gparam) : 0.f;
      }
      *reinterpret_cast<float4*>(dx + (size_t)b * in + i) = make_float4(d[0], d[1], d[2], d[3]);
    }
    }
  }
#pragma unroll
  for (int e = 0; e < 4; ++e)
#pragma unroll
    for (int o = 0; o < OUT; ++o) dw[(i + e) * OUT + o] = acc[e][o];
}

__global__ void colsum_small_kernel(const float* __restrict__ dy, float* __restrict__ db, int B, int out) {
  const int o = threadIdx.x;
  if (o >= out) return;
  float s = 0.f;
  for (int b = 0; b < B; ++b) s += dy[(size_t)b * out + o];
  db[o] = s;
}

int dense_small_bwd(const float* x, const float* w, const float* dy, float* dx, float* dw, float* db, int B, int in, int out, hipStream_t s, int gact,
                    float gparam, const uint8_t* gmask, float gscale) {
  if (out < 1 || out > 4 || in % 4) {
    set_error("dense_small_bwd: out %d (1..4) / in %d (%%4) unsupported", out, in);
    return GN_EINVAL;
  }
  const unsigned grid = cdiv((size_t)in / 4, 256);
  switch (out) {
    case 1: hipLaunchKernelGGL(dense_small_bwd_kernel<1>, dim3(grid), dim3(256), 0, s, x, w, dy, dx, dw, B, in, gact, gparam, gmask, gscale); break;
    case 2: hipLaunchKernelGGL(dense_small_bwd_kernel<2>, dim3(grid), dim3(256), 0, s, x, w, dy, dx, dw, B, in, gact, gparam, gmask, gscale); break;
    case 3: hipLaunchKernelGGL(dense_small_bwd_kernel<3>, dim3(grid), dim3(256), 0, s, x, w, dy, dx, dw, B, in, gact, gparam, gmask, gscale); break;
    default: hipLaunchKernelGGL(dense_small_bwd_kernel<4>, dim3(grid), dim3(256), 0, s, x, w, dy, dx, dw, B, in, gact, gparam, gmask, gscale); break;
  }
  int rc = check_launch("dense_small_bwd");
  if (rc) return rc;
  if (db) {
    hipLaunchKernelGGL(colsum_small_kernel, dim3(1), dim3(64), 0, s, dy, db, B, out);
    rc = check_launch("colsum_small");
  }
  return rc;
}

}
```

### gennet_amd/csrc/wgrad_wino.hip

```cpp
#include <stdlib.h>
#include <algorithm>
#include <type_traits>
#include "common.h"
#include "wino_common.h"

namespace gn {

template <int O>
__device__ __forceinline__ void wg_slot_e(f32x4& c, float a, float b, f32x2& e0, f32x2& e1, unsigned addr_b) {
  asm volatile(
      "ds_read2st64_b32 %1, %5 offset0:%6 offset1:%7\n\t"
      "ds_read2st64_b32 %2, %5 offset0:%8 offset1:%9\n\t"
      "v_mfma_f32_16x16x4_f32 %0, %3, %4, %0"
      : "+v"(c), "=&v"(e0), "=&v"(e1)
      : "v"(a), "v"(b), "v"(addr_b), "i"(O), "i"(O + 1), "i"(O + 4), "i"(O + 5)
      : "memory");
}
template <int O, int OA>
__device__ __forceinline__ void wg_slot_ea(f32x4& c, float a, float b, f32x2& e0, f32x2& e1, unsigned addr_b, f32x2 (&d)[6], const unsigned (&addr_a)[3]) {
  asm volatile(
      "ds_read2st64_b32 %1, %11 offset0:%15 offset1:%16\n\t"
      "ds_read2st64_b32 %2, %11 offset0:%17 offset1:%18\n\t"
      "ds_read2st64_b32 %3, %12 offset0:%19 offset1:%20\n\t"
      "ds_read2st64_b32 %4, %12 offset0:%21 offset1:%22\n\t"
      "ds_read2st64_b32 %5, %13 offset0:%19 offset1:%20\n\t"
      "ds_read2st64_b32 %6, %13 offset0:%21 offset1:%22\n\t"
      "ds_read2st64_b32 %7, %14 offset0:%19 offset1:%20\n\t"
      "ds_read2st64_b32 %8, %14 offset0:%21 offset1:%22\n\t"
      "v_mfma_f32_16x16x4_f32 %0, %9, %10, %0"
      : "+v"(c), "=&v"(e0), "=&v"(e1), "=&v"(d[0]), "=&v"(d[1]), "=&v"(d[2]), "=&v"(d[3]), "=&v"(d[4]), "=&v"(d[5])
      : "v"(a), "v"(b), "v"(addr_b), "v"(addr_a[0]), "v"(addr_a[1]), "v"(addr_a[2]), "i"(O), "i"(O + 1), "i"(O + 4), "i"(O + 5), "i"(OA), "i"(OA + 1), "i"(OA + 5),
        "i"(OA + 6)
      : "memory");
}
template <int O>
__device__ __forceinline__ void wg_slot_e_wd(f32x4& c, float a, float b, f32x2& e0, f32x2& e1, unsigned addr_b, f32x2 (&d)[6]) {
  asm volatile(
      "ds_read2st64_b32 %1, %11 offset0:%12 offset1:%13\n\t"
      "ds_read2st64_b32 %2, %11 offset0:%14 offset1:%15\n\t"
      "s_waitcnt lgkmcnt(2)\n\t"
      "v_mfma_f32_16x16x4_f32 %0, %9, %10, %0"
      : "+v"(c), "=&v"(e0), "=&v"(e1), "+v"(d[0]), "+v"(d[1]), "+v"(d[2]), "+v"(d[3]), "+v"(d[4]), "+v"(d[5])
      : "v"(a), "v"(b), "v"(addr_b), "i"(O), "i"(O + 1), "i"(O + 4), "i"(O + 5)
      : "memory");
}

template <int H, int ABL = 0>
struct WgPair {
  template <int NP0, int NP1, int I = 0, class DMA>
  static __device__ __forceinline__ void run(f32x4 (&acc)[6][4], const f32x2 (&v)[6], f32x2 (&vn)[6], f32x2 (&d)[6], WinoT& t, f32x2 (&D)[2][6], unsigned addr_b,
                                             unsigned addr_b_next, const unsigned (&addr_a)[3], const unsigned (&addr_a_next)[3], unsigned long long k15,
                                             unsigned long long km15, DMA& dma) {
    if constexpr (I < 48) {
      constexpr int CT = I / 12, G = I % 12, S = G / 6, P = G % 6;
      f32x2(&dc)[6] = D[CT & 1];
      f32x2(&dn)[6] = D[(CT + 1) & 1];
      const float av = v[P][S], bv = dc[P][S];
      constexpr int OE = (CT < 3) ? (CT + 1) * 8 + 2 * H : (H == 0 ? 2 : 0);
      if constexpr ((ABL & 8) != 0) wino_slot(acc[P][CT], av, bv);
      else if constexpr (I == 0) {
        if constexpr (H == 0) wg_slot_ea<OE, 2>(acc[P][CT], av, bv, dn[0], dn[5], addr_b, d, addr_a);
        else wg_slot_ea<OE, 0>(acc[P][CT], av, bv, dn[0], dn[5], addr_b, d, addr_a_next);
      } else if constexpr (I == 12) wg_slot_e_wd<OE>(acc[P][CT], av, bv, dn[0], dn[5], addr_b, d);
      else if constexpr (G == 0) {
        if constexpr (CT == 3 && H == 1) wg_slot_e<OE>(acc[P][CT], av, bv, dn[0], dn[5], addr_b_next);
        else wg_slot_e<OE>(acc[P][CT], av, bv, dn[0], dn[5], addr_b);
      } else if constexpr (G == 4) wino_slot_w<(I == 4 ? 6 : 0)>(acc[P][CT], av, bv, dn[0], dn[5]);
      else wino_slot(acc[P][CT], av, bv);
      if constexpr (G == 4) {
        constexpr int K = (H == 0 ? 0 : NP0) + CT;
        if constexpr (CT < (H == 0 ? NP0 : NP1)) dma(std::integral_constant<int, K>{});
      }
      if constexpr (!(ABL & 2)) {
        if constexpr (G == 5) {
          wino_a_piece<0>(dn[0], dn[5], dn[1], dn[2], dn[3], dn[4]); wino_a_piece<1>(dn[0], dn[5], dn[1], dn[2], dn[3], dn[4]);
          wino_a_piece<2>(dn[0], dn[5], dn[1], dn[2], dn[3], dn[4]); wino_a_piece<3>(dn[0], dn[5], dn[1], dn[2], dn[3], dn[4]);
        }
        if constexpr (CT == 1 && G == 9) wino_run<0, 5>(d, vn, t, k15, km15);
        if constexpr (CT == 2 && G == 9) wino_run<5, 10>(d, vn, t, k15, km15);
        if constexpr (CT == 3 && G == 9) wino_run<10, kWinoPieces>(d, vn, t, k15, km15);
      }
      run<NP0, NP1, I + 1>(acc, v, vn, d, t, D, addr_b, addr_b_next, addr_a, addr_a_next, k15, km15, dma);
    }
  }
};

template <int ABL = 0>
__global__ __launch_bounds__(256, 2) void wgrad_wino_kernel(WgradArgs a, int off0, int cpb) {
#if defined(__HIP_DEVICE_COMPILE__)
  constexpr int NT = 256;
  constexpr int XS = 4 * 2 * 20 * 16;
  constexpr int YS = 4 * 2 * 16 * 16;
  constexpr int BUF = XS + YS;
  constexpr int STAGE_BYTES = BUF * 4;
  extern __shared__ __attribute__((aligned(16))) float smem[];
  typedef __attribute__((address_space(3))) void* lptr_t;

  const int tid = threadIdx.x, lane = tid & 63, wave = tid >> 6;
  const int n16 = lane & 15, kq = lane >> 4;
  const int ci0 = blockIdx.x * 64, co0 = blockIdx.y * 64, split = blockIdx.z;
  const int total = a.B * cpb;
  const int q_begin = split * a.chunks_per_split, q_end = min(q_begin + a.chunks_per_split, total);

  f32x4 acc[6][4];
#pragma unroll
  for (int p = 0; p < 6; ++p)
#pragma unroll
    for (int ct = 0; ct < 4; ++ct)
#pragma unroll
      for (int r = 0; r < 4; ++r) acc[p][ct][r] = 0.f;

  constexpr int X_ITEMS = 3, Y_ITEMS = 2;
  int xoff[X_ITEMS], yoff[Y_ITEMS];
#pragma unroll
  for (int it = 0; it < X_ITEMS; ++it) {
    const int g = tid + it * NT;
    const int sub = g / 160, rem = g % 160, plane = rem / 80, prow = (rem % 80) >> 2, c4 = rem & 3;
    xoff[it] = ((2 * prow + plane + off0) * a.Cin + ci0 + sub * 16 + 4 * c4) * 4;
  }
#pragma unroll
  for (int it = 0; it < Y_ITEMS; ++it) {
    const int g = tid + it * NT;
    const int ct = g >> 7, rem = g & 127, plane = rem >> 6, tile = (rem & 63) >> 2, c4 = rem & 3;
    yoff[it] = ((2 * tile + plane) * a.Cout + co0 + ct * 16 + 4 * c4) * 4;
  }
  const int xbytes = __builtin_amdgcn_readfirstlane(a.Lin * a.Cin * 4), ybytes = __builtin_amdgcn_readfirstlane(a.M * a.Cout * 4);
  int q_next = 0, st_next = 0;
  bool in_loop = false;
  const int wv64 = __builtin_amdgcn_readfirstlane(tid & ~63);
  auto dma_piece = [&](auto kc) {
    constexpr int k = decltype(kc)::value;
    if ((ABL & 1) && in_loop) return;
    const int b = __builtin_amdgcn_readfirstlane(q_next / cpb), cb = __builtin_amdgcn_readfirstlane(q_next % cpb);
    float* stg = smem + st_next * BUF;
    if constexpr (k < X_ITEMS) {
      if (k < 2 || wv64 < 128) {
        const uintptr_t p = (uintptr_t)(a.x + (size_t)b * a.Lin * a.Cin);
        const __amdgpu_buffer_rsrc_t srd = __builtin_amdgcn_make_buffer_rsrc((void*)p, 0, xbytes, 0x00020000);
        gn_buffer_load_lds(srd, (lptr_t)(stg + (k * NT + wv64) * 4), 16, xoff[k] + cb * 32 * a.Cin * 4, 0, 0, 0);
      }
    } else {
      constexpr int it = k - X_ITEMS;
      const int cbo = cb * 32 * a.Cout * 4;
      const uintptr_t p = (uintptr_t)(a.dy + (size_t)b * a.M * a.Cout) + (uintptr_t)(unsigned)cbo;
      const __amdgpu_buffer_rsrc_t srd = __builtin_amdgcn_make_buffer_rsrc((void*)p, 0, ybytes - cbo, 0x00020000);
      gn_buffer_load_lds(srd, (lptr_t)(stg + XS + (it * NT + wv64) * 4), 16, yoff[it], 0, 0, 0);
    }
  };
  auto dma_all = [&]() {
    dma_piece(std::integral_constant<int, 0>{}); dma_piece(std::integral_constant<int, 1>{}); dma_piece(std::integral_constant<int, 2>{});
    dma_piece(std::integral_constant<int, 3>{}); dma_piece(std::integral_constant<int, 4>{});
  };

  const unsigned lds0 = (unsigned)(uintptr_t)smem;
  unsigned base_a[3];
#pragma unroll
  for (int j2 = 0; j2 < 3; ++j2) base_a[j2] = lds0 + wave * 2560 + ((kq + j2) * 16 + n16) * 4;
  const unsigned base_b = lds0 + XS * 4 + (kq * 16 + n16) * 4;
  const unsigned long long k15 = 0x3fc000003fc00000ull, km15 = 0xbfc00000bfc00000ull;

  if (q_begin < q_end) {
    q_next = q_begin; st_next = 0; dma_all();
    q_next = min(q_begin + 1, q_end - 1); st_next = 1; dma_all();
    __syncthreads();

    f32x2 V0[6], V1[6], d[6], D[2][6];
    WinoT tt;
    {
      const char* sb = reinterpret_cast<const char*>(smem);
#pragma unroll
      for (int j = 0; j < 6; ++j) {
        const float* pp = reinterpret_cast<const float*>(sb + (base_a[j >> 1] - lds0) + (j & 1) * 1280);
        d[j][0] = pp[0]; d[j][1] = pp[64];
      }
      wino_run<0, kWinoPieces>(d, V0, tt, k15, km15);
      const float* pb = reinterpret_cast<const float*>(sb + (base_b - lds0));
      D[0][0][0] = pb[0]; D[0][0][1] = pb[64]; D[0][5][0] = pb[256]; D[0][5][1] = pb[320];
      wino_a_piece<0>(D[0][0], D[0][5], D[0][1], D[0][2], D[0][3], D[0][4]); wino_a_piece<1>(D[0][0], D[0][5], D[0][1], D[0][2], D[0][3], D[0][4]);
      wino_a_piece<2>(D[0][0], D[0][5], D[0][1], D[0][2], D[0][3], D[0][4]); wino_a_piece<3>(D[0][0], D[0][5], D[0][1], D[0][2], D[0][3], D[0][4]);
    }
    int st = 0;
    in_loop = true;
    for (int q = q_begin; q < q_end; ++q) {
      const int st1 = st == 2 ? 0 : st + 1, st2 = st1 == 2 ? 0 : st1 + 1;
      q_next = min(q + 2, q_end - 1);
      st_next = st2;
      unsigned addr_a[3], addr_a_next[3];
#pragma unroll
      for (int j2 = 0; j2 < 3; ++j2) { addr_a[j2] = base_a[j2] + st * STAGE_BYTES; addr_a_next[j2] = base_a[j2] + st1 * STAGE_BYTES; }
      const unsigned addr_b = base_b + st * STAGE_BYTES, addr_b_next = base_b + st1 * STAGE_BYTES;
      WgPair<0, ABL>::template run<3, 2>(acc, V0, V1, d, tt, D, addr_b, addr_b_next, addr_a, addr_a_next, k15, km15, dma_piece);
      WgPair<1, ABL>::template run<3, 2>(acc, V1, V0, d, tt, D, addr_b, addr_b_next, addr_a, addr_a_next, k15, km15, dma_piece);
      if constexpr (!(ABL & 4)) __syncthreads();
      st = st1;
    }
    asm volatile("s_nop 15\n\ts_nop 7" : "+v"(acc[5][0]), "+v"(acc[5][1]), "+v"(acc[5][2]), "+v"(acc[5][3]));
  }

  const size_t cc = (size_t)a.Cin * a.Cout;
#pragma unroll
  for (int p = 0; p < 6; ++p) {
    float* dst = a.part + ((size_t)split * 6 + p) * cc + (size_t)(ci0 + wave * 16 + 4 * kq) * a.Cout + co0 + n16;
#pragma unroll
    for (int ct = 0; ct < 4; ++ct)
#pragma unroll
      for (int r = 0; r < 4; ++r) dst[(size_t)r * a.Cout + ct * 16] = acc[p][ct][r];
  }
#endif
}

__global__ void wgrad_wino_reduce_kernel(const float* __restrict__ part, float* __restrict__ dw, size_t cc, int splits) {
  const size_t i = (size_t)blockIdx.x * blockDim.x + threadIdx.x;
  if (i >= cc) return;
  double Q[6] = {0, 0, 0, 0, 0, 0};
#pragma unroll 4
  for (int s = 0; s < splits; ++s)
#pragma unroll
    for (int p = 0; p < 6; ++p) Q[p] += (double)part[((size_t)s * 6 + p) * cc + i];
  const double e = (Q[1] + Q[2]) * (1.0 / 3.0), o = (Q[1] - Q[2]) * (1.0 / 3.0);
  dw[i] = (float)(Q[0] + e + Q[3] * (16.0 / 15.0) + Q[4] * (1.0 / 30.0));
  dw[cc + i] = (float)(o + Q[3] * (8.0 / 15.0) - Q[4] * (2.0 / 30.0));
  dw[2 * cc + i] = (float)(e + Q[3] * (4.0 / 15.0) + Q[4] * (4.0 / 30.0));
  dw[3 * cc + i] = (float)(o + Q[3] * (2.0 / 15.0) - Q[4] * (8.0 / 30.0));
  dw[4 * cc + i] = (float)(e + Q[3] * (1.0 / 15.0) + Q[4] * (16.0 / 30.0) + Q[5]);
}

bool wgrad_wino_supported(const WgradArgs& a) {
  if (a.ntaps != 5 || a.in_stride != 1 || a.Cin % 64 || a.Cout % 64) return false;
  for (int j = 0; j < 5; ++j)
    if (a.off[j] != a.off[0] + j) return false;
  return (size_t)a.Lin * a.Cin * 4 < 0x40000000ull && (size_t)a.M * a.Cout * 4 < 0x40000000ull;
}

size_t wgrad_wino_workspace_bytes(int B, int M, int Cin, int Cout) {
  int s, cps;
  wgrad_split_plan(B, M, Cin, Cout, 64, 64, &s, &cps);
  return (size_t)s * 6 * Cin * Cout * sizeof(float);
}

int wgrad_wino_run(WgradArgs& a, float* dw, hipStream_t s) {
  if (!wgrad_wino_supported(a)) {
    set_error("wgrad_wino: unsupported shape");
    return GN_EINVAL;
  }
  int splits;
  wgrad_split_plan(a.B, a.M, a.Cin, a.Cout, 64, 64, &splits, &a.chunks_per_split);
  const int cpb = (a.M + 31) / 32;
  constexpr size_t lds = 3 * sizeof(float) * (4 * 2 * 20 * 16 + 4 * 2 * 16 * 16);
  dim3 grid(a.Cin / 64, a.Cout / 64, splits);
  prof_begin(s);
#ifdef GN_ABLATION
  static const int abl = getenv("GN_WGWINO_ABL") ? atoi(getenv("GN_WGWINO_ABL")) : 0;
  if (abl == 1) hipLaunchKernelGGL(wgrad_wino_kernel<1>, grid, dim3(256), lds, s, a, a.off[0], cpb);
  else if (abl == 2) hipLaunchKernelGGL(wgrad_wino_kernel<2>, grid, dim3(256), lds, s, a, a.off[0], cpb);
  else if (abl == 8) hipLaunchKernelGGL(wgrad_wino_kernel<8>, grid, dim3(256), lds, s, a, a.off[0], cpb);
  else if (abl == 15) hipLaunchKernelGGL(wgrad_wino_kernel<15>, grid, dim3(256), lds, s, a, a.off[0], cpb);
  else
#endif
  hipLaunchKernelGGL(wgrad_wino_kernel<0>, grid, dim3(256), lds, s, a, a.off[0], cpb);
  prof_end(s, 0.6 * 2.0 * a.B * (double)a.M * 5 * a.Cin * a.Cout, 6, 4.0 * ((double)a.B * a.Lin * a.Cin + (double)a.B * a.M * a.Cout + 5.0 * a.Cin * a.Cout));
  int rc = check_launch("wgrad_wino");
  if (rc) return rc;
  const size_t cc = (size_t)a.Cin * a.Cout;
  hipLaunchKernelGGL(wgrad_wino_reduce_kernel, dim3(cdiv(cc, 256)), dim3(256), 0, s, a.part, dw, cc, splits);
  return check_launch("wgrad_wino_reduce");
}

}
```

### gennet_amd/csrc/wgrad_wino_s2.hip

```cpp
#include <stdlib.h>
#include <algorithm>
#include <type_traits>
#include "common.h"
#include "wino_common.h"

namespace gn {

template <int O>
__device__ __forceinline__ void wg2_slot_e(f32x4& c, float a, float b, f32x2& e0, f32x2& e1, unsigned addr_b) {
  asm volatile(
      "ds_read2st64_b32 %1, %5 offset0:%6 offset1:%7\n\t"
      "ds_read2st64_b32 %2, %5 offset0:%8 offset1:%9\n\t"
      "v_mfma_f32_16x16x4_f32 %0, %3, %4, %0"
      : "+v"(c), "=&v"(e0), "=&v"(e1)
      : "v"(a), "v"(b), "v"(addr_b), "i"(O), "i"(O + 1), "i"(O + 2), "i"(O + 3)
      : "memory");
}
template <int O>
__device__ __forceinline__ void wg2_slot_ea(f32x4& c, float a, float b, f32x2& e0, f32x2& e1, unsigned addr_b, f32x2 (&d)[7], const unsigned (&addr_a)[2]) {
  asm volatile(
      "ds_read2st64_b32 %1, %12 offset0:%15 offset1:%16\n\t"
      "ds_read2st64_b32 %2, %12 offset0:%17 offset1:%18\n\t"
      "ds_read2st64_b32 %3, %13 offset0:0 offset1:1\n\t"
      "ds_read2st64_b32 %4, %13 offset0:3 offset1:4\n\t"
      "ds_read2st64_b32 %5, %13 offset0:6 offset1:7\n\t"
      "ds_read2st64_b32 %6, %13 offset0:9 offset1:10\n\t"
      "ds_read2st64_b32 %7, %14 offset0:0 offset1:1\n\t"
      "ds_read2st64_b32 %8, %14 offset0:3 offset1:4\n\t"
      "ds_read2st64_b32 %9, %14 offset0:6 offset1:7\n\t"
      "v_mfma_f32_16x16x4_f32 %0, %10, %11, %0"
      : "+v"(c), "=&v"(e0), "=&v"(e1), "=&v"(d[0]), "=&v"(d[1]), "=&v"(d[2]), "=&v"(d[3]), "=&v"(d[4]), "=&v"(d[5]), "=&v"(d[6])
      : "v"(a), "v"(b), "v"(addr_b), "v"(addr_a[0]), "v"(addr_a[1]), "i"(O), "i"(O + 1), "i"(O + 2), "i"(O + 3)
      : "memory");
}
template <int O>
__device__ __forceinline__ void wg2_slot_e_wd(f32x4& c, float a, float b, f32x2& e0, f32x2& e1, unsigned addr_b, f32x2 (&d)[7]) {
  asm volatile(
      "ds_read2st64_b32 %1, %12 offset0:%13 offset1:%14\n\t"
      "ds_read2st64_b32 %2, %12 offset0:%15 offset1:%16\n\t"
      "s_waitcnt lgkmcnt(2)\n\t"
      "v_mfma_f32_16x16x4_f32 %0, %10, %11, %0"
      : "+v"(c), "=&v"(e0), "=&v"(e1), "+v"(d[0]), "+v"(d[1]), "+v"(d[2]), "+v"(d[3]), "+v"(d[4]), "+v"(d[5]), "+v"(d[6])
      : "v"(a), "v"(b), "v"(addr_b), "i"(O), "i"(O + 1), "i"(O + 2), "i"(O + 3)
      : "memory");
}

struct Wg2Chunk {
  template <int NPIECES, int I = 0, class DMA>
  static __device__ __forceinline__ void run(f32x4 (&acc)[7][4], const f32x2 (&v)[7], f32x2 (&vn)[7], f32x2 (&d)[7], f32x2 (&D)[2][4], unsigned addr_b,
                                             unsigned addr_b_next, const unsigned (&addr_a_next)[2], DMA& dma) {
    if constexpr (I < 56) {
      constexpr int CT = I / 14, G = I % 14, S = G / 7, P = G % 7;
      constexpr int BI = (P == 0 || P == 4) ? 0 : ((P == 1 || P == 5) ? 2 : (P == 2 ? 3 : 1));
      f32x2(&dc)[4] = D[CT & 1];
      f32x2(&dn)[4] = D[(CT + 1) & 1];
      const float av = v[P][S], bv = dc[BI][S];
      constexpr int OE = (CT < 3) ? (CT + 1) * 4 : 0;
      if constexpr (I == 0) wg2_slot_ea<OE>(acc[P][CT], av, bv, dn[0], dn[1], addr_b, d, addr_a_next);
      else if constexpr (I == 14) wg2_slot_e_wd<OE>(acc[P][CT], av, bv, dn[0], dn[1], addr_b, d);
      else if constexpr (G == 0) {
        if constexpr (CT == 3) wg2_slot_e<OE>(acc[P][CT], av, bv, dn[0], dn[1], addr_b_next);
        else wg2_slot_e<OE>(acc[P][CT], av, bv, dn[0], dn[1], addr_b);
      } else if constexpr (G == 4) wino_slot_w<(I == 4 ? 7 : 0)>(acc[P][CT], av, bv, dn[0], dn[1]);
      else wino_slot(acc[P][CT], av, bv);
      if constexpr (G == 4 && CT < NPIECES) dma(std::integral_constant<int, CT>{});
      if constexpr (G == 5) {
        GN_PK_ADD(dn[2], dn[0], dn[1]);
        GN_PK_SUB(dn[3], dn[0], dn[1]);
      }
      if constexpr (CT == 1 && G == 9) s2_run<1, 0, 7, 0, 4>(d, vn);
      if constexpr (CT == 2 && G == 9) s2_run<1, 0, 7, 4, 7>(d, vn);
      run<NPIECES, I + 1>(acc, v, vn, d, D, addr_b, addr_b_next, addr_a_next, dma);
    }
  }
};

__global__ __launch_bounds__(256, 2) void wgrad_wino_s2_kernel(WgradArgs a, int off0, int cpb) {
#if defined(__HIP_DEVICE_COMPILE__)
  constexpr int NT = 256;
  constexpr int XS = 4 * 4 * 12 * 16;
  constexpr int YS = 4 * 2 * 8 * 16;
  constexpr int BUF = XS + YS;
  constexpr int STAGE_BYTES = BUF * 4;
  extern __shared__ __attribute__((aligned(16))) float smem[];
  typedef __attribute__((address_space(3))) void* lptr_t;

  const int tid = threadIdx.x, lane = tid & 63, wave = tid >> 6;
  const int n16 = lane & 15, kq = lane >> 4;
  const int ci0 = blockIdx.x * 64, co0 = blockIdx.y * 64, split = blockIdx.z;
  const int total = a.B * cpb;
  const int q_begin = split * a.chunks_per_split, q_end = min(q_begin + a.chunks_per_split, total);

  f32x4 acc[7][4];
#pragma unroll
  for (int p = 0; p < 7; ++p)
#pragma unroll
    for (int ct = 0; ct < 4; ++ct)
#pragma unroll
      for (int r = 0; r < 4; ++r) acc[p][ct][r] = 0.f;

  constexpr int X_ITEMS = 3;
  int xoff[X_ITEMS], yoff;
#pragma unroll
  for (int it = 0; it < X_ITEMS; ++it) {
    const int g = tid + it * NT;
    const int sub = g / 192, rem = g % 192, plane = rem / 48, prow = (rem % 48) >> 2, c4 = rem & 3;
    xoff[it] = ((4 * prow + plane + off0) * a.Cin + ci0 + sub * 16 + 4 * c4) * 4;
  }
  {
    const int g = tid;
    const int ct = g >> 6, rem = g & 63, plane = rem >> 5, tile = (rem & 31) >> 2, c4 = rem & 3;
    yoff = ((2 * tile + plane) * a.Cout + co0 + ct * 16 + 4 * c4) * 4;
  }
  const int xbytes = __builtin_amdgcn_readfirstlane(a.Lin * a.Cin * 4), ybytes = __builtin_amdgcn_readfirstlane(a.M * a.Cout * 4);
  int q_next = 0, st_next = 0;
  const int wv64 = __builtin_amdgcn_readfirstlane(tid & ~63);
  auto dma_piece = [&](auto kc) {
    constexpr int k = decltype(kc)::value;
    const int b = __builtin_amdgcn_readfirstlane(q_next / cpb), cb = __builtin_amdgcn_readfirstlane(q_next % cpb);
    float* stg = smem + st_next * BUF;
    if constexpr (k < X_ITEMS) {
      const uintptr_t p = (uintptr_t)(a.x + (size_t)b * a.Lin * a.Cin);
      const __amdgpu_buffer_rsrc_t srd = __builtin_amdgcn_make_buffer_rsrc((void*)p, 0, xbytes, 0x00020000);
      gn_buffer_load_lds(srd, (lptr_t)(stg + (k * NT + wv64) * 4), 16, xoff[k] + cb * 32 * a.Cin * 4, 0, 0, 0);
    } else {
      const int cbo = cb * 16 * a.Cout * 4;
      const uintptr_t p = (uintptr_t)(a.dy + (size_t)b * a.M * a.Cout) + (uintptr_t)(unsigned)cbo;
      const __amdgpu_buffer_rsrc_t srd = __builtin_amdgcn_make_buffer_rsrc((void*)p, 0, ybytes - cbo, 0x00020000);
      gn_buffer_load_lds(srd, (lptr_t)(stg + XS + wv64 * 4), 16, yoff, 0, 0, 0);
    }
  };
  auto dma_all = [&]() {
    dma_piece(std::integral_constant<int, 0>{}); dma_piece(std::integral_constant<int, 1>{}); dma_piece(std::integral_constant<int, 2>{});
    dma_piece(std::integral_constant<int, 3>{});
  };

  const unsigned lds0 = (unsigned)(uintptr_t)smem;
  unsigned base_a[2];
#pragma unroll
  for (int j4 = 0; j4 < 2; ++j4) base_a[j4] = lds0 + wave * 3072 + ((kq + j4) * 16 + n16) * 4;
  const unsigned base_b = lds0 + XS * 4 + (kq * 16 + n16) * 4;

  if (q_begin < q_end) {
    q_next = q_begin; st_next = 0; dma_all();
    q_next = min(q_begin + 1, q_end - 1); st_next = 1; dma_all();
    __syncthreads();

    f32x2 V0[7], V1[7], d[7], D[2][4];
    {
      const char* sb = reinterpret_cast<const char*>(smem);
#pragma unroll
      for (int j = 0; j < 7; ++j) {
        const float* pp = reinterpret_cast<const float*>(sb + (base_a[j >> 2] - lds0) + (j & 3) * 768);
        d[j][0] = pp[0]; d[j][1] = pp[64];
      }
      s2_run<1, 0, 7, 0, 7>(d, V0);
      const float* pb = reinterpret_cast<const float*>(sb + (base_b - lds0));
      D[0][0][0] = pb[0]; D[0][0][1] = pb[64]; D[0][1][0] = pb[128]; D[0][1][1] = pb[192];
      GN_PK_ADD(D[0][2], D[0][0], D[0][1]);
      GN_PK_SUB(D[0][3], D[0][0], D[0][1]);
    }
    int st = 0;
    for (int q = q_begin; q < q_end; q += 2) {
#pragma unroll
      for (int half = 0; half < 2; ++half) {
        if (half == 1 && q + 1 >= q_end) break;
        const int st1 = st == 2 ? 0 : st + 1, st2 = st1 == 2 ? 0 : st1 + 1;
        q_next = min(q + half + 2, q_end - 1);
        st_next = st2;
        unsigned addr_a_next[2];
#pragma unroll
        for (int j4 = 0; j4 < 2; ++j4) addr_a_next[j4] = base_a[j4] + st1 * STAGE_BYTES;
        const unsigned addr_b = base_b + st * STAGE_BYTES, addr_b_next = base_b + st1 * STAGE_BYTES;
        if (half == 0) Wg2Chunk::run<4>(acc, V0, V1, d, D, addr_b, addr_b_next, addr_a_next, dma_piece);
        else Wg2Chunk::run<4>(acc, V1, V0, d, D, addr_b, addr_b_next, addr_a_next, dma_piece);
        __syncthreads();
        st = st1;
      }
    }
    asm volatile("s_nop 15\n\ts_nop 7" : "+v"(acc[6][0]), "+v"(acc[6][1]), "+v"(acc[6][2]), "+v"(acc[6][3]));
  }

  const size_t cc = (size_t)a.Cin * a.Cout;
#pragma unroll
  for (int p = 0; p < 7; ++p) {
    float* dst = a.part + ((size_t)split * 7 + p) * cc + (size_t)(ci0 + wave * 16 + 4 * kq) * a.Cout + co0 + n16;
#pragma unroll
    for (int ct = 0; ct < 4; ++ct)
#pragma unroll
      for (int r = 0; r < 4; ++r) dst[(size_t)r * a.Cout + ct * 16] = acc[p][ct][r];
  }
#endif
}

__global__ void wgrad_wino_s2_reduce_kernel(const float* __restrict__ part, float* __restrict__ dw, size_t cc, int splits) {
  const size_t i = (size_t)blockIdx.x * blockDim.x + threadIdx.x;
  if (i >= cc) return;
  double Q[7] = {0, 0, 0, 0, 0, 0, 0};
#pragma unroll 4
  for (int s = 0; s < splits; ++s)
#pragma unroll
    for (int p = 0; p < 7; ++p) Q[p] += (double)part[((size_t)s * 7 + p) * cc + i];
  dw[i] = (float)(Q[0] + 0.5 * (Q[1] + Q[2]));
  dw[cc + i] = (float)(Q[4] + Q[5]);
  dw[2 * cc + i] = (float)(0.5 * (Q[1] - Q[2]));
  dw[3 * cc + i] = (float)(Q[5] + Q[6]);
  dw[4 * cc + i] = (float)(0.5 * (Q[1] + Q[2]) - Q[3]);
}

static void s2_plan(int B, int M, int Cin, int Cout, int* splits, int* cps16, int* cpb16) {
  int s, cps32;
  wgrad_split_plan(B, M, Cin, Cout, 64, 64, &s, &cps32);
  *cpb16 = (M + 15) / 16;
  const int cpb32 = (M + 31) / 32;
  if (cps32 % cpb32 == 0) *cps16 = (cps32 / cpb32) * *cpb16;
  else *cps16 = 2 * cps32;
  const long total = (long)B * *cpb16;
  *splits = (int)((total + *cps16 - 1) / *cps16);
}

bool wgrad_wino_s2_supported(const WgradArgs& a) {
  if (a.ntaps != 5 || a.in_stride != 2 || a.Cin % 64 || a.Cout % 64) return false;
  for (int j = 0; j < 5; ++j)
    if (a.off[j] != a.off[0] + j) return false;
  return (size_t)a.Lin * a.Cin * 4 < 0x40000000ull && (size_t)a.M * a.Cout * 4 < 0x40000000ull;
}

size_t wgrad_wino_s2_workspace_bytes(int B, int M, int Cin, int Cout) {
  int s, cps, cpb;
  s2_plan(B, M, Cin, Cout, &s, &cps, &cpb);
  return (size_t)s * 7 * Cin * Cout * sizeof(float);
}

int wgrad_wino_s2_run(WgradArgs& a, float* dw, hipStream_t s) {
  if (!wgrad_wino_s2_supported(a)) {
    set_error("wgrad_wino_s2: unsupported shape");
    return GN_EINVAL;
  }
  int splits, cpb;
  s2_plan(a.B, a.M, a.Cin, a.Cout, &splits, &a.chunks_per_split, &cpb);
  constexpr size_t lds = 3 * sizeof(float) * (4 * 4 * 12 * 16 + 4 * 2 * 8 * 16);
  dim3 grid(a.Cin / 64, a.Cout / 64, splits);
  prof_begin(s);
  hipLaunchKernelGGL(wgrad_wino_s2_kernel, grid, dim3(256), lds, s, a, a.off[0], cpb);
  prof_end(s, 0.7 * 2.0 * a.B * (double)a.M * 5 * a.Cin * a.Cout, 8, 4.0 * ((double)a.B * a.Lin * a.Cin + (double)a.B * a.M * a.Cout + 5.0 * a.Cin * a.Cout));
  int rc = check_launch("wgrad_wino_s2");
  if (rc) return rc;
  const size_t cc = (size_t)a.Cin * a.Cout;
  hipLaunchKernelGGL(wgrad_wino_s2_reduce_kernel, dim3(cdiv(cc, 256)), dim3(256), 0, s, a.part, dw, cc, splits);
  return check_launch("wgrad_wino_s2_reduce");
}

}
```

### gennet_amd/csrc/wino_common.h

```cpp
#pragma once
#include "common.h"

namespace gn {

typedef float f32x4 __attribute__((ext_vector_type(4)));
typedef float f32x2 __attribute__((ext_vector_type(2)));

struct WinoT {
  f32x2 a, b;
};
constexpr int kWinoPieces = 14;
#define GN_PK_ADD(o, x, y) asm volatile("v_pk_add_f32 %0, %1, %2" : "=&v"(o) : "v"(x), "v"(y))
#define GN_PK_COPY(o, x) asm volatile("v_pk_mul_f32 %0, %1, 1.0 op_sel_hi:[1,0]" : "=&v"(o) : "v"(x))
#define GN_PK_SUB(o, x, y) asm volatile("v_pk_add_f32 %0, %1, %2 neg_lo:[0,1] neg_hi:[0,1]" : "=&v"(o) : "v"(x), "v"(y))
#define GN_PK_SUB_SELF(o, y) asm volatile("v_pk_add_f32 %0, %0, %1 neg_lo:[0,1] neg_hi:[0,1]" : "+v"(o) : "v"(y))
#define GN_PK_ADD_SELF(o, y) asm volatile("v_pk_add_f32 %0, %0, %1" : "+v"(o) : "v"(y))
#define GN_PK_FMA_NEW(o, x, c, z) asm volatile("v_pk_fma_f32 %0, %1, " c ", %2 op_sel_hi:[1,0,1]" : "=&v"(o) : "v"(x), "v"(z))
#define GN_PK_FMA_SELF(o, c, z) asm volatile("v_pk_fma_f32 %0, %0, " c ", %1 op_sel_hi:[1,0,1]" : "+v"(o) : "v"(z))
#define GN_PK_FMA_NEWS_NEG(o, x, k, z) asm volatile("v_pk_fma_f32 %0, %1, %2, %3 neg_lo:[0,0,1] neg_hi:[0,0,1]" : "=&v"(o) : "v"(x), "s"(k), "v"(z))
#define GN_PK_FMA_ACCS(o, x, k) asm volatile("v_pk_fma_f32 %0, %1, %2, %0" : "+v"(o) : "v"(x), "s"(k))
template <int K>
__device__ __forceinline__ void wino_piece(const f32x2 (&d)[6], f32x2 (&v)[6], WinoT& t, unsigned long long k15, unsigned long long km15) {
  if constexpr (K == 0) GN_PK_SUB(t.a, d[1], d[3]);
  else if constexpr (K == 1) GN_PK_SUB(t.b, d[2], d[4]);
  else if constexpr (K == 2) GN_PK_SUB(v[0], d[0], d[2]);
  else if constexpr (K == 3) GN_PK_SUB(v[5], d[5], d[3]);
  else if constexpr (K == 4) GN_PK_FMA_NEWS_NEG(v[1], d[2], k15, t.a);
  else if constexpr (K == 5) GN_PK_FMA_NEWS_NEG(v[2], d[3], k15, t.b);
  else if constexpr (K == 6) GN_PK_FMA_NEW(v[3], t.a, "2.0", t.b);
  else if constexpr (K == 7) GN_PK_FMA_NEW(v[4], t.b, "-2.0", t.a);
  else if constexpr (K == 8) GN_PK_SUB_SELF(v[0], t.b);
  else if constexpr (K == 9) GN_PK_ADD_SELF(v[5], t.a);
  else if constexpr (K == 10) GN_PK_FMA_ACCS(v[0], t.a, km15);
  else if constexpr (K == 11) GN_PK_FMA_ACCS(v[5], t.b, km15);
  else if constexpr (K == 12) GN_PK_ADD_SELF(v[1], v[2]);
  else if constexpr (K == 13) GN_PK_FMA_SELF(v[2], "-2.0", v[1]);
}
template <int K0, int K1>
__device__ __forceinline__ void wino_run(const f32x2 (&d)[6], f32x2 (&v)[6], WinoT& t, unsigned long long k15, unsigned long long km15) {
  if constexpr (K0 < K1) {
    wino_piece<K0>(d, v, t, k15, km15);
    wino_run<K0 + 1, K1>(d, v, t, k15, km15);
  }
}

template <int KIND, int SB, int K, int NR>
__device__ __forceinline__ void s2_piece(const f32x2 (&d)[NR], f32x2 (&v)[7]) {
  constexpr int A0 = 0, A1 = KIND == 1 ? 2 : 1, A2 = KIND == 1 ? 4 : 2, A3 = KIND == 1 ? 6 : 3;
  constexpr int B0 = KIND == 1 ? 1 : SB, B1 = KIND == 1 ? 3 : SB + 1, B2 = KIND == 1 ? 5 : SB + 2;
  if constexpr (K == 0) GN_PK_SUB(v[0], d[A0], d[A2]);
  else if constexpr (K == 1) GN_PK_ADD(v[1], d[A1], d[A2]);
  else if constexpr (K == 2) GN_PK_SUB(v[2], d[A2], d[A1]);
  else if constexpr (K == 3) GN_PK_SUB(v[3], d[A1], d[A3]);
  else if constexpr (K == 4) GN_PK_SUB(v[4], d[B0], d[B1]);
  else if constexpr (K == 5) GN_PK_COPY(v[5], d[B1]);
  else GN_PK_SUB(v[6], d[B2], d[B1]);
}
template <int KIND, int SB, int NR, int K0, int K1>
__device__ __forceinline__ void s2_run(const f32x2 (&d)[NR], f32x2 (&v)[7]) {
  if constexpr (K0 < K1) {
    s2_piece<KIND, SB, K0, NR>(d, v);
    s2_run<KIND, SB, NR, K0 + 1, K1>(d, v);
  }
}

__device__ __forceinline__ void wino_slot(f32x4& c, float a, float b) {
  asm volatile("v_mfma_f32_16x16x4_f32 %0, %1, %2, %0" : "+v"(c) : "v"(a), "v"(b) : "memory");
}
template <int O, int WAIT>
__device__ __forceinline__ void wino_slot_rb(f32x4& c, float a, float b, f32x4& nb0, f32x4& nb1, unsigned addr_b) {
  asm volatile(
      "ds_read_b128 %1, %5 offset:%6\n\t"
      "ds_read_b128 %2, %5 offset:%7\n\t"
      "s_waitcnt lgkmcnt(%8)\n\t"
      "v_mfma_f32_16x16x4_f32 %0, %3, %4, %0"
      : "+v"(c), "=&v"(nb0), "=&v"(nb1)
      : "v"(a), "v"(b), "v"(addr_b), "i"(O), "i"(O + 1024), "i"(WAIT)
      : "memory");
}
template <int WAIT>
__device__ __forceinline__ void wino_slot_w(f32x4& c, float a, float b, f32x2& e0, f32x2& e1) {
  asm volatile("s_waitcnt lgkmcnt(%5)\n\tv_mfma_f32_16x16x4_f32 %0, %3, %4, %0" : "+v"(c), "+v"(e0), "+v"(e1) : "v"(a), "v"(b), "i"(WAIT) : "memory");
}


template <int K>
__device__ __forceinline__ void wino_a_piece(const f32x2& e0, const f32x2& e1, f32x2& p1, f32x2& p2, f32x2& p3, f32x2& p4) {
  if constexpr (K == 0) GN_PK_ADD(p1, e0, e1);
  else if constexpr (K == 1) GN_PK_SUB(p2, e0, e1);
  else if constexpr (K == 2) GN_PK_FMA_NEW(p3, e1, "0.5", e0);
  else GN_PK_FMA_NEW(p4, e1, "-2.0", e0);
}

}
```

Measured before the change: 1950.

## Fuse bias-gradient reduction into small and Winograd wgrad kernels

The small-channel wgrad kernel and the Winograd wgrad kernels (stride 1 and stride 2) now accumulate the bias gradient from the dy tiles they already load. Each writes per-split double partials, which the existing reduce kernels finalize, so the separate bias_grad pass that re-read dy is dropped. The cost is a little extra LDS traffic and f64 adds inside the tight MFMA schedules, plus a larger workspace and an extra barrier for the block reduction.

```diff
diff --git a/gennet_amd/csrc/capi.hip b/gennet_amd/csrc/capi.hip
--- a/gennet_amd/csrc/capi.hip
+++ b/gennet_amd/csrc/capi.hip
@@ -483,7 +483,9 @@
     case WGRAD_SMALL: {
       WgradSmallArgs sa = {x, dy, (float*)ws, B, L, Cin, Cout, Lout, k, stride};
       std::copy(a.off, a.off + k, sa.off);
-      rc = wgrad_small_dispatch(sa, dw, ws_bytes, s);
+      bool done = false;
+      rc = wgrad_small_dispatch(sa, dw, ws_bytes, s, db, &done);
+      a.db_done = done;
       break;
     }
     case WGRAD_WINO: rc = wgrad_wino_run(a, dw, s); break;
@@ -495,9 +497,9 @@
       break;
     default:
       rc = wgrad_mfma_dispatch(a, dw, ws_bytes, s);
-      if (!rc && a.db_done) return GN_OK;
   }
   if (rc) return rc;
+  if (a.db_done) return GN_OK;
   return db ? bias_grad(dy, db, (size_t)B * Lout, Cout, ws, ws_bytes, s) : GN_OK;
 }
 
diff --git a/gennet_amd/csrc/common.h b/gennet_amd/csrc/common.h
--- a/gennet_amd/csrc/common.h
+++ b/gennet_amd/csrc/common.h
@@ -79,6 +79,7 @@
   int ntaps, in_stride;
   int off[8];
   int rows_per_chunk;
+  double* db_part;
 };
 
 struct LazyDy {
@@ -142,7 +143,7 @@
 int conv_smallcin_dispatch(const ConvArgs& a, hipStream_t s);
 int conv_smallcout_dispatch(const ConvArgs& a, hipStream_t s);
 size_t wgrad_small_workspace_bytes(int B, int M, int Cin, int Cout, int ntaps);
-int wgrad_small_dispatch(WgradSmallArgs a, float* dw, size_t ws_bytes, hipStream_t s);
+int wgrad_small_dispatch(WgradSmallArgs a, float* dw, size_t ws_bytes, hipStream_t s, float* db = nullptr, bool* db_done = nullptr);
 int dense_small_fwd(const float* x, const float* w, const float* bias, float* y, int B, int in, int out, int act, float p, hipStream_t s);
 int dense_small_bwd(const float* x, const float* w, const float* dy, float* dx, float* dw, float* db, int B, int in, int out, hipStream_t s,
                     int gact = 0, float gparam = 0.f, const uint8_t* gmask = nullptr, float gscale = 1.f);
diff --git a/gennet_amd/csrc/small_conv.hip b/gennet_amd/csrc/small_conv.hip
--- a/gennet_amd/csrc/small_conv.hip
+++ b/gennet_amd/csrc/small_conv.hip
@@ -231,6 +231,8 @@
     for (int c = 0; c < CS; ++c) acc[j][c] = make_float4(0.f, 0.f, 0.f, 0.f);
   __shared__ float tab[TR][MAXT * CS];
   __shared__ float4 red[256];
+  const bool do_bias = a.db_part != nullptr;
+  double bs[4] = {0.0, 0.0, 0.0, 0.0};
 
   const size_t rows = (size_t)a.B * a.M;
   const size_t r_lo = (size_t)blockIdx.y * a.rows_per_chunk;
@@ -256,6 +258,12 @@
           const int rr = r0 + u * RL;
           g[u] = rr < nr ? *reinterpret_cast<const float4*>(a.dy + (base + rr) * a.Cout + 4 * q) : make_float4(0.f, 0.f, 0.f, 0.f);
         }
+        if (do_bias) {
+#pragma unroll
+          for (int u = 0; u < U; ++u) {
+            bs[0] += (double)g[u].x; bs[1] += (double)g[u].y; bs[2] += (double)g[u].z; bs[3] += (double)g[u].w;
+          }
+        }
 #pragma unroll
         for (int u = 0; u < U; ++u) {
           const int rr = r0 + u * RL;
@@ -290,6 +298,20 @@
         }
         float* pc = a.part + (size_t)blockIdx.y * a.ntaps * a.Cin * a.Cout;
         *reinterpret_cast<float4*>(pc + ((size_t)j * CS + c) * a.Cout + 4 * q) = s;
+      }
+    }
+  }
+  if (do_bias) {
+    double* redb = reinterpret_cast<double*>(red);
+#pragma unroll
+    for (int e = 0; e < 4; ++e) {
+      __syncthreads();
+      redb[tid] = bs[e];
+      __syncthreads();
+      if (rl == 0 && q < NQ) {
+        double t = redb[ql];
+        for (int k = 1; k < RL; ++k) t += redb[k * NQc + ql];
+        a.db_part[(size_t)blockIdx.y * a.Cout + 4 * q + e] = t;
       }
     }
   }
@@ -472,7 +494,8 @@
 
 size_t wgrad_small_workspace_bytes(int B, int M, int Cin, int Cout, int ntaps) {
   const int CL = Cin <= 4 ? Cout : Cin;
-  return (size_t)wgrad_small_chunks((size_t)B * M, CL) * ntaps * Cin * Cout * sizeof(float);
+  const size_t chunks = (size_t)wgrad_small_chunks((size_t)B * M, CL);
+  return chunks * ntaps * Cin * Cout * sizeof(float) + (Cin <= 4 ? chunks * Cout * sizeof(double) : 0);
 }
 
 constexpr int SUM_GROUPS = 32;
@@ -505,7 +528,7 @@
   return check_launch("wgrad_small_reduce");
 }
 
-int wgrad_small_dispatch(WgradSmallArgs a, float* dw, size_t ws_bytes, hipStream_t s) {
+int wgrad_small_dispatch(WgradSmallArgs a, float* dw, size_t ws_bytes, hipStream_t s, float* db, bool* db_done) {
   const bool small_in = a.Cin <= 4;
   const int CS = small_in ? a.Cin : a.Cout, CL = small_in ? a.Cout : a.Cin;
   if (CS < 1 || CS > 4 || CL % 4 || a.ntaps > 5) {
@@ -514,7 +537,7 @@
   }
   const size_t rows = (size_t)a.B * a.M;
   const int chunks = wgrad_small_chunks(rows, CL);
-  if (ws_bytes < (size_t)chunks * a.ntaps * a.Cin * a.Cout * sizeof(float)) {
+  if (ws_bytes < wgrad_small_workspace_bytes(a.B, a.M, a.Cin, a.Cout, a.ntaps)) {
     set_error("wgrad_small: workspace too small");
     return GN_EWORKSPACE;
   }
@@ -534,6 +557,7 @@
     const size_t n1 = (size_t)a.ntaps * a.Cin * a.Cout;
     return sum_partials(a.part, dw, n1, chunks, s);
   }
+  a.db_part = small_in && db ? reinterpret_cast<double*>(a.part + (size_t)chunks * a.ntaps * a.Cin * a.Cout) : nullptr;
 #define GN_WS(CSV)                                                                                            \
   if (small_in) hipLaunchKernelGGL((wgrad_smallcin_tab_kernel<CSV>), grid, dim3(256), 0, s, a);               \
   else hipLaunchKernelGGL((wgrad_small_kernel<CSV, false>), grid, dim3(256), 0, s, a);
@@ -547,7 +571,11 @@
   int rc = check_launch("wgrad_small");
   if (rc) return rc;
   const size_t n = (size_t)a.ntaps * a.Cin * a.Cout;
-  return sum_partials(a.part, dw, n, chunks, s);
+  rc = sum_partials(a.part, dw, n, chunks, s);
+  if (rc || !a.db_part) return rc;
+  rc = colred_finalize_f32(a.db_part, db, (size_t)a.Cout, chunks, s);
+  if (!rc && db_done) *db_done = true;
+  return rc;
 }
 
 template <int OUT>
diff --git a/gennet_amd/csrc/wgrad_wino.hip b/gennet_amd/csrc/wgrad_wino.hip
--- a/gennet_amd/csrc/wgrad_wino.hip
+++ b/gennet_amd/csrc/wgrad_wino.hip
@@ -50,13 +50,16 @@
   template <int NP0, int NP1, int I = 0, class DMA>
   static __device__ __forceinline__ void run(f32x4 (&acc)[6][4], const f32x2 (&v)[6], f32x2 (&vn)[6], f32x2 (&d)[6], WinoT& t, f32x2 (&D)[2][6], unsigned addr_b,
                                              unsigned addr_b_next, const unsigned (&addr_a)[3], const unsigned (&addr_a_next)[3], unsigned long long k15,
-                                             unsigned long long km15, DMA& dma) {
+                                             unsigned long long km15, DMA& dma, WgBias<4>& bias) {
     if constexpr (I < 48) {
       constexpr int CT = I / 12, G = I % 12, S = G / 6, P = G % 6;
       f32x2(&dc)[6] = D[CT & 1];
       f32x2(&dn)[6] = D[(CT + 1) & 1];
       const float av = v[P][S], bv = dc[P][S];
       constexpr int OE = (CT < 3) ? (CT + 1) * 8 + 2 * H : (H == 0 ? 2 : 0);
+      if constexpr (H == 0 && I == 0 && ABL == 0) {
+        if (bias.on) wg_bias_read(bias);
+      }
       if constexpr ((ABL & 8) != 0) wino_slot(acc[P][CT], av, bv);
       else if constexpr (I == 0) {
         if constexpr (H == 0) wg_slot_ea<OE, 2>(acc[P][CT], av, bv, dn[0], dn[5], addr_b, d, addr_a);
@@ -75,12 +78,15 @@
         if constexpr (G == 5) {
           wino_a_piece<0>(dn[0], dn[5], dn[1], dn[2], dn[3], dn[4]); wino_a_piece<1>(dn[0], dn[5], dn[1], dn[2], dn[3], dn[4]);
           wino_a_piece<2>(dn[0], dn[5], dn[1], dn[2], dn[3], dn[4]); wino_a_piece<3>(dn[0], dn[5], dn[1], dn[2], dn[3], dn[4]);
+          if constexpr (H == 0 && I == 5 && ABL == 0) {
+            if (bias.on) wg_bias_add(bias);
+          }
         }
         if constexpr (CT == 1 && G == 9) wino_run<0, 5>(d, vn, t, k15, km15);
         if constexpr (CT == 2 && G == 9) wino_run<5, 10>(d, vn, t, k15, km15);
         if constexpr (CT == 3 && G == 9) wino_run<10, kWinoPieces>(d, vn, t, k15, km15);
       }
-      run<NP0, NP1, I + 1>(acc, v, vn, d, t, D, addr_b, addr_b_next, addr_a, addr_a_next, k15, km15, dma);
+      run<NP0, NP1, I + 1>(acc, v, vn, d, t, D, addr_b, addr_b_next, addr_a, addr_a_next, k15, km15, dma, bias);
     }
   }
 };
@@ -159,6 +165,12 @@
   const unsigned base_b = lds0 + XS * 4 + (kq * 16 + n16) * 4;
   const unsigned long long k15 = 0x3fc000003fc00000ull, km15 = 0xbfc00000bfc00000ull;
 
+  WgBias<4> bias;
+  bias.on = a.db_part != nullptr && blockIdx.x == 0;
+  bias.sum = 0.0;
+#pragma unroll
+  for (int i = 0; i < 4; ++i) bias.z[i] = f32x2{0.f, 0.f};
+
   if (q_begin < q_end) {
     q_next = q_begin; st_next = 0; dma_all();
     q_next = min(q_begin + 1, q_end - 1); st_next = 1; dma_all();
@@ -189,13 +201,15 @@
 #pragma unroll
       for (int j2 = 0; j2 < 3; ++j2) { addr_a[j2] = base_a[j2] + st * STAGE_BYTES; addr_a_next[j2] = base_a[j2] + st1 * STAGE_BYTES; }
       const unsigned addr_b = base_b + st * STAGE_BYTES, addr_b_next = base_b + st1 * STAGE_BYTES;
-      WgPair<0, ABL>::template run<3, 2>(acc, V0, V1, d, tt, D, addr_b, addr_b_next, addr_a, addr_a_next, k15, km15, dma_piece);
-      WgPair<1, ABL>::template run<3, 2>(acc, V1, V0, d, tt, D, addr_b, addr_b_next, addr_a, addr_a_next, k15, km15, dma_piece);
+      bias.addr = addr_b + wave * 2048;
+      WgPair<0, ABL>::template run<3, 2>(acc, V0, V1, d, tt, D, addr_b, addr_b_next, addr_a, addr_a_next, k15, km15, dma_piece, bias);
+      WgPair<1, ABL>::template run<3, 2>(acc, V1, V0, d, tt, D, addr_b, addr_b_next, addr_a, addr_a_next, k15, km15, dma_piece, bias);
       if constexpr (!(ABL & 4)) __syncthreads();
       st = st1;
     }
     asm volatile("s_nop 15\n\ts_nop 7" : "+v"(acc[5][0]), "+v"(acc[5][1]), "+v"(acc[5][2]), "+v"(acc[5][3]));
   }
+  if (bias.on) wg_bias_store(bias.sum, smem, a.db_part + (size_t)split * a.Cout + co0);
 
   const size_t cc = (size_t)a.Cin * a.Cout;
 #pragma unroll
@@ -209,9 +223,11 @@
 #endif
 }
 
-__global__ void wgrad_wino_reduce_kernel(const float* __restrict__ part, float* __restrict__ dw, size_t cc, int splits) {
+__global__ void wgrad_wino_reduce_kernel(const float* __restrict__ part, float* __restrict__ dw, size_t cc, int splits, const double* __restrict__ db_part,
+                                         float* __restrict__ db, int Cout) {
   const size_t i = (size_t)blockIdx.x * blockDim.x + threadIdx.x;
   if (i >= cc) return;
+  wgrad_wino_reduce_bias(db_part, db, Cout, splits, i);
   double Q[6] = {0, 0, 0, 0, 0, 0};
 #pragma unroll 4
   for (int s = 0; s < splits; ++s)
@@ -235,7 +251,7 @@
 size_t wgrad_wino_workspace_bytes(int B, int M, int Cin, int Cout) {
   int s, cps;
   wgrad_split_plan(B, M, Cin, Cout, 64, 64, &s, &cps);
-  return (size_t)s * 6 * Cin * Cout * sizeof(float);
+  return (size_t)s * 6 * Cin * Cout * sizeof(float) + (size_t)s * Cout * sizeof(double);
 }
 
 int wgrad_wino_run(WgradArgs& a, float* dw, hipStream_t s) {
@@ -248,6 +264,8 @@
   const int cpb = (a.M + 31) / 32;
   constexpr size_t lds = 3 * sizeof(float) * (4 * 2 * 20 * 16 + 4 * 2 * 16 * 16);
   dim3 grid(a.Cin / 64, a.Cout / 64, splits);
+  const size_t cc = (size_t)a.Cin * a.Cout;
+  a.db_part = a.db ? reinterpret_cast<double*>(a.part + (size_t)splits * 6 * cc) : nullptr;
   prof_begin(s);
 #ifdef GN_ABLATION
   static const int abl = getenv("GN_WGWINO_ABL") ? atoi(getenv("GN_WGWINO_ABL")) : 0;
@@ -261,9 +279,10 @@
   prof_end(s, 0.6 * 2.0 * a.B * (double)a.M * 5 * a.Cin * a.Cout, 6, 4.0 * ((double)a.B * a.Lin * a.Cin + (double)a.B * a.M * a.Cout + 5.0 * a.Cin * a.Cout));
   int rc = check_launch("wgrad_wino");
   if (rc) return rc;
-  const size_t cc = (size_t)a.Cin * a.Cout;
-  hipLaunchKernelGGL(wgrad_wino_reduce_kernel, dim3(cdiv(cc, 256)), dim3(256), 0, s, a.part, dw, cc, splits);
-  return check_launch("wgrad_wino_reduce");
-}
-
-}
+  hipLaunchKernelGGL(wgrad_wino_reduce_kernel, dim3(cdiv(cc, 256)), dim3(256), 0, s, a.part, dw, cc, splits, a.db_part, a.db, a.Cout);
+  rc = check_launch("wgrad_wino_reduce");
+  if (!rc && a.db_part) a.db_done = 1;
+  return rc;
+}
+
+}
diff --git a/gennet_amd/csrc/wgrad_wino_s2.hip b/gennet_amd/csrc/wgrad_wino_s2.hip
--- a/gennet_amd/csrc/wgrad_wino_s2.hip
+++ b/gennet_amd/csrc/wgrad_wino_s2.hip
@@ -48,7 +48,7 @@
 struct Wg2Chunk {
   template <int NPIECES, int I = 0, class DMA>
   static __device__ __forceinline__ void run(f32x4 (&acc)[7][4], const f32x2 (&v)[7], f32x2 (&vn)[7], f32x2 (&d)[7], f32x2 (&D)[2][4], unsigned addr_b,
-                                             unsigned addr_b_next, const unsigned (&addr_a_next)[2], DMA& dma) {
+                                             unsigned addr_b_next, const unsigned (&addr_a_next)[2], DMA& dma, WgBias<2>& bias) {
     if constexpr (I < 56) {
       constexpr int CT = I / 14, G = I % 14, S = G / 7, P = G % 7;
       constexpr int BI = (P == 0 || P == 4) ? 0 : ((P == 1 || P == 5) ? 2 : (P == 2 ? 3 : 1));
@@ -56,6 +56,9 @@
       f32x2(&dn)[4] = D[(CT + 1) & 1];
       const float av = v[P][S], bv = dc[BI][S];
       constexpr int OE = (CT < 3) ? (CT + 1) * 4 : 0;
+      if constexpr (I == 0) {
+        if (bias.on) wg_bias_read(bias);
+      }
       if constexpr (I == 0) wg2_slot_ea<OE>(acc[P][CT], av, bv, dn[0], dn[1], addr_b, d, addr_a_next);
       else if constexpr (I == 14) wg2_slot_e_wd<OE>(acc[P][CT], av, bv, dn[0], dn[1], addr_b, d);
       else if constexpr (G == 0) {
@@ -67,10 +70,13 @@
       if constexpr (G == 5) {
         GN_PK_ADD(dn[2], dn[0], dn[1]);
         GN_PK_SUB(dn[3], dn[0], dn[1]);
+        if constexpr (I == 5) {
+          if (bias.on) wg_bias_add(bias);
+        }
       }
       if constexpr (CT == 1 && G == 9) s2_run<1, 0, 7, 0, 4>(d, vn);
       if constexpr (CT == 2 && G == 9) s2_run<1, 0, 7, 4, 7>(d, vn);
-      run<NPIECES, I + 1>(acc, v, vn, d, D, addr_b, addr_b_next, addr_a_next, dma);
+      run<NPIECES, I + 1>(acc, v, vn, d, D, addr_b, addr_b_next, addr_a_next, dma, bias);
     }
   }
 };
@@ -141,6 +147,11 @@
   for (int j4 = 0; j4 < 2; ++j4) base_a[j4] = lds0 + wave * 3072 + ((kq + j4) * 16 + n16) * 4;
   const unsigned base_b = lds0 + XS * 4 + (kq * 16 + n16) * 4;
 
+  WgBias<2> bias;
+  bias.on = a.db_part != nullptr && blockIdx.x == 0;
+  bias.sum = 0.0;
+  bias.z[0] = bias.z[1] = f32x2{0.f, 0.f};
+
   if (q_begin < q_end) {
     q_next = q_begin; st_next = 0; dma_all();
     q_next = min(q_begin + 1, q_end - 1); st_next = 1; dma_all();
@@ -172,14 +183,16 @@
 #pragma unroll
         for (int j4 = 0; j4 < 2; ++j4) addr_a_next[j4] = base_a[j4] + st1 * STAGE_BYTES;
         const unsigned addr_b = base_b + st * STAGE_BYTES, addr_b_next = base_b + st1 * STAGE_BYTES;
-        if (half == 0) Wg2Chunk::run<4>(acc, V0, V1, d, D, addr_b, addr_b_next, addr_a_next, dma_piece);
-        else Wg2Chunk::run<4>(acc, V1, V0, d, D, addr_b, addr_b_next, addr_a_next, dma_piece);
+        bias.addr = addr_b + wave * 1024;
+        if (half == 0) Wg2Chunk::run<4>(acc, V0, V1, d, D, addr_b, addr_b_next, addr_a_next, dma_piece, bias);
+        else Wg2Chunk::run<4>(acc, V1, V0, d, D, addr_b, addr_b_next, addr_a_next, dma_piece, bias);
         __syncthreads();
         st = st1;
       }
     }
     asm volatile("s_nop 15\n\ts_nop 7" : "+v"(acc[6][0]), "+v"(acc[6][1]), "+v"(acc[6][2]), "+v"(acc[6][3]));
   }
+  if (bias.on) wg_bias_store(bias.sum, smem, a.db_part + (size_t)split * a.Cout + co0);
 
   const size_t cc = (size_t)a.Cin * a.Cout;
 #pragma unroll
@@ -193,9 +206,11 @@
 #endif
 }
 
-__global__ void wgrad_wino_s2_reduce_kernel(const float* __restrict__ part, float* __restrict__ dw, size_t cc, int splits) {
+__global__ void wgrad_wino_s2_reduce_kernel(const float* __restrict__ part, float* __restrict__ dw, size_t cc, int splits, const double* __restrict__ db_part,
+                                            float* __restrict__ db, int Cout) {
   const size_t i = (size_t)blockIdx.x * blockDim.x + threadIdx.x;
   if (i >= cc) return;
+  wgrad_wino_reduce_bias(db_part, db, Cout, splits, i);
   double Q[7] = {0, 0, 0, 0, 0, 0, 0};
 #pragma unroll 4
   for (int s = 0; s < splits; ++s)
@@ -229,7 +244,7 @@
 size_t wgrad_wino_s2_workspace_bytes(int B, int M, int Cin, int Cout) {
   int s, cps, cpb;
   s2_plan(B, M, Cin, Cout, &s, &cps, &cpb);
-  return (size_t)s * 7 * Cin * Cout * sizeof(float);
+  return (size_t)s * 7 * Cin * Cout * sizeof(float) + (size_t)s * Cout * sizeof(double);
 }
 
 int wgrad_wino_s2_run(WgradArgs& a, float* dw, hipStream_t s) {
@@ -241,14 +256,17 @@
   s2_plan(a.B, a.M, a.Cin, a.Cout, &splits, &a.chunks_per_split, &cpb);
   constexpr size_t lds = 3 * sizeof(float) * (4 * 4 * 12 * 16 + 4 * 2 * 8 * 16);
   dim3 grid(a.Cin / 64, a.Cout / 64, splits);
+  const size_t cc = (size_t)a.Cin * a.Cout;
+  a.db_part = a.db ? reinterpret_cast<double*>(a.part + (size_t)splits * 7 * cc) : nullptr;
   prof_begin(s);
   hipLaunchKernelGGL(wgrad_wino_s2_kernel, grid, dim3(256), lds, s, a, a.off[0], cpb);
   prof_end(s, 0.7 * 2.0 * a.B * (double)a.M * 5 * a.Cin * a.Cout, 8, 4.0 * ((double)a.B * a.Lin * a.Cin + (double)a.B * a.M * a.Cout + 5.0 * a.Cin * a.Cout));
   int rc = check_launch("wgrad_wino_s2");
   if (rc) return rc;
-  const size_t cc = (size_t)a.Cin * a.Cout;
-  hipLaunchKernelGGL(wgrad_wino_s2_reduce_kernel, dim3(cdiv(cc, 256)), dim3(256), 0, s, a.part, dw, cc, splits);
-  return check_launch("wgrad_wino_s2_reduce");
-}
-
-}
+  hipLaunchKernelGGL(wgrad_wino_s2_reduce_kernel, dim3(cdiv(cc, 256)), dim3(256), 0, s, a.part, dw, cc, splits, a.db_part, a.db, a.Cout);
+  rc = check_launch("wgrad_wino_s2_reduce");
+  if (!rc && a.db_part) a.db_done = 1;
+  return rc;
+}
+
+}
diff --git a/gennet_amd/csrc/wino_common.h b/gennet_amd/csrc/wino_common.h
--- a/gennet_amd/csrc/wino_common.h
+++ b/gennet_amd/csrc/wino_common.h
@@ -83,6 +83,63 @@
   asm volatile("s_waitcnt lgkmcnt(%5)\n\tv_mfma_f32_16x16x4_f32 %0, %3, %4, %0" : "+v"(c), "+v"(e0), "+v"(e1) : "v"(a), "v"(b), "i"(WAIT) : "memory");
 }
 
+template <int N>
+struct WgBias {
+  f32x2 z[N];
+  double sum;
+  unsigned addr;
+  bool on;
+};
+template <int N>
+__device__ __forceinline__ void wg_bias_read(WgBias<N>& b) {
+  static_assert(N == 2 || N == 4, "one or two 1 KiB row planes of two tiles each");
+  if constexpr (N == 2)
+    asm volatile(
+        "ds_read2st64_b32 %0, %2 offset0:0 offset1:1\n\t"
+        "ds_read2st64_b32 %1, %2 offset0:2 offset1:3"
+        : "=&v"(b.z[0]), "=&v"(b.z[1])
+        : "v"(b.addr)
+        : "memory");
+  else
+    asm volatile(
+        "ds_read2st64_b32 %0, %4 offset0:0 offset1:1\n\t"
+        "ds_read2st64_b32 %1, %4 offset0:2 offset1:3\n\t"
+        "ds_read2st64_b32 %2, %4 offset0:4 offset1:5\n\t"
+        "ds_read2st64_b32 %3, %4 offset0:6 offset1:7"
+        : "=&v"(b.z[0]), "=&v"(b.z[1]), "=&v"(b.z[2]), "=&v"(b.z[3])
+        : "v"(b.addr)
+        : "memory");
+}
+template <int N>
+__device__ __forceinline__ void wg_bias_add(WgBias<N>& b) {
+  double t0, t1;
+#pragma unroll
+  for (int i = 0; i < N; ++i)
+    asm volatile(
+        "v_cvt_f64_f32 %1, %3\n\t"
+        "v_cvt_f64_f32 %2, %4\n\t"
+        "v_add_f64 %0, %0, %1\n\t"
+        "v_add_f64 %0, %0, %2"
+        : "+v"(b.sum), "=&v"(t0), "=&v"(t1)
+        : "v"(b.z[i][0]), "v"(b.z[i][1]));
+}
+__device__ __forceinline__ void wg_bias_store(double sum, float* smem, double* db_part_row) {
+  double* red = reinterpret_cast<double*>(smem);
+  const int tid = threadIdx.x;
+  red[tid] = sum;
+  __syncthreads();
+  if (tid < 64) {
+    const double* r = red + (tid >> 4) * 64 + (tid & 15);
+    db_part_row[tid] = ((r[0] + r[16]) + r[32]) + r[48];
+  }
+}
+__device__ __forceinline__ void wgrad_wino_reduce_bias(const double* __restrict__ db_part, float* __restrict__ db, int Cout, int splits, size_t i) {
+  if (db_part == nullptr || i >= (size_t)Cout) return;
+  double t = 0.0;
+  for (int s = 0; s < splits; ++s) t += db_part[(size_t)s * Cout + i];
+  db[i] = (float)t;
+}
+
 
 template <int K>
 __device__ __forceinline__ void wino_a_piece(const f32x2& e0, const f32x2& e1, f32x2& p1, f32x2& p2, f32x2& p3, f32x2& p4) {
```

Result: no change. 1964, median of 6 (+0.7%).
